# ColinWine/Multi-modal-Multi-label-Facial-Action-Unit-Detection-with-Transformer

Hardware: NVIDIA B200
Metric: AVFormer hot-path clips/sec (forward) (higher is better)
Workload: dtype bf16

## Files before the change

multi-modal-multi-label-facial-action-unit-detection-with-transformer_b200/csrc/avf_api.cu:

```cuda
#include <atomic>
#include <cstdarg>
#include <cstdio>
#include <cstring>

#include "avf_common.cuh"
#include "avf_internal.h"

namespace avf {

static thread_local char g_err[512] = "";
static std::atomic<uint64_t> g_launches{0};
static std::atomic<int> g_pdl{1};
bool pdl_enabled() { return g_pdl.load() != 0; }
static std::atomic<int> g_sm_cap{0};
int sm_cap() { return g_sm_cap.load(); }
static std::atomic<int> g_fused{1};

void count_launch() { g_launches.fetch_add(1, std::memory_order_relaxed); }

void set_error(const char* fmt, ...) {
  va_list ap;
  va_start(ap, fmt);
  vsnprintf(g_err, sizeof(g_err), fmt, ap);
  va_end(ap);
}

int check_cuda(cudaError_t e, const char* what) {
  if (e == cudaSuccess) return 0;
  set_error("CUDA error %d (%s) at %s", int(e), cudaGetErrorString(e), what);
  return int(e);
}

static int require_device() {
  static int state = 0;
  if (state == 0) {
    int n = 0;
    cudaError_t e = cudaGetDeviceCount(&n);
    if (e != cudaSuccess || n == 0) {
      cudaGetLastError();
      state = -1;
    } else {
      state = 1;
    }
  }
  if (state < 0) {
    set_error("no CUDA device: the AVFormer B200 path has no CPU fallback");
    return AVF_ENODEVICE;
  }
  return 0;
}

static bool tcgen05_ok() {
  static int state = 0;
  if (state == 0) {
    int dev = 0, major = 0;
    if (cudaGetDevice(&dev) == cudaSuccess && cudaDeviceGetAttribute(&major, cudaDevAttrComputeCapabilityMajor, dev) == cudaSuccess)
      state = (major == 10) ? 1 : -1;
    else
      state = -1;
  }
  return state > 0;
}

static inline size_t align_up(size_t v, size_t a = 256) { return (v + a - 1) / a * a; }
static inline size_t elt(int mode) { return mode == AVF_BF16 ? 2 : 4; }

struct EncoderWs {
  void* ln;
  void* qkv;
  void* attn;
  void* hid;
  size_t total;
};

static EncoderWs carve_encoder_ws(const avf_stack_shape* s, int mode, void* base) {
  const size_t R = size_t(s->n_seq) * s->n_tok, I = size_t(s->heads) * s->dim_head, e = elt(mode);
  uint8_t* p = static_cast<uint8_t*>(base);
  EncoderWs w;
  size_t off = 0;
  w.ln = p + off;   off += align_up(R * s->dim * e);
  w.qkv = p + off;  off += align_up(R * 3 * I * e);
  w.attn = p + off; off += align_up(R * I * e);
  w.hid = p + off;  off += align_up(R * s->mlp_dim * e);
  w.total = off;
  return w;
}

static int check_shape(const avf_stack_shape* s) {
  AVF_REQUIRE(s != nullptr, AVF_EINVAL, "null stack shape");
  AVF_REQUIRE(s->n_seq > 0 && s->n_tok > 0 && s->depth > 0, AVF_EINVAL, "empty stack: n_seq=%d n_tok=%d depth=%d", s->n_seq, s->n_tok, s->depth);
  AVF_REQUIRE(s->dim % 128 == 0 && s->dim <= 1536, AVF_EUNSUPPORTED, "dim=%d must be a multiple of 128 (<= 1536)", s->dim);
  AVF_REQUIRE(s->dim_head == 32 || s->dim_head == 64, AVF_EUNSUPPORTED, "dim_head=%d (supported: 32, 64)", s->dim_head);
  AVF_REQUIRE((s->heads * s->dim_head) % 64 == 0 && s->mlp_dim % 64 == 0, AVF_EUNSUPPORTED, "inner=%d / mlp=%d must be multiples of 64", s->heads * s->dim_head, s->mlp_dim);
  AVF_REQUIRE(s->n_tok <= 64 || s->dim_head == 64, AVF_EUNSUPPORTED,
              "n_tok=%d: sequences longer than 64 tokens are not part of this path for dim_head=%d", s->n_tok, s->dim_head);
  AVF_REQUIRE(s->n_tok <= 256, AVF_EUNSUPPORTED, "n_tok=%d: sequences longer than 256 tokens are not part of this path", s->n_tok);
  return 0;
}

int linear(int mode, const void* a, int lda, const void* w, const float* bias, const float* res, int ld_res, void* c, int ldc,
           int c_mode, int m, int n, int k, int flags, cudaStream_t st) {
  if (mode == AVF_BF16) {
    AVF_REQUIRE(tcgen05_ok(), AVF_EUNSUPPORTED, "bf16 mode needs an sm_100 device (tcgen05)");
    return linear_umma(a, lda, w, bias, res, ld_res, c, ldc, c_mode, m, n, k, flags, st);
  }
  return linear_f32(static_cast<const float*>(a), lda, static_cast<const float*>(w), bias, res, ld_res, c, ldc, c_mode, m, n, k, flags, st);
}

static bool fused_rows(int mode, const avf_stack_shape* s, int ld_x, const float* out, int ld_out) {
  return mode == AVF_BF16 && g_fused.load() && tcgen05_ok() && encoder_fused_supported(s) &&
         ld_x % 4 == 0 && (out == nullptr || ld_out % 4 == 0);
}

static int encoder_stack(int mode, const avf_stack_shape* s, const avf_layer_weights* L, float* x, int ld_x, float* out, int ld_out,
                         void* ws, size_t ws_bytes, cudaStream_t st, const uint8_t* keep = nullptr) {
  int e = check_shape(s);
  if (e) return e;
  AVF_REQUIRE(mode == AVF_BF16 || mode == AVF_FP32, AVF_EINVAL, "mode=%d", mode);
  AVF_REQUIRE(L != nullptr && x != nullptr && ws != nullptr, AVF_EINVAL, "null pointer argument");
  if (keep == nullptr && fused_rows(mode, s, ld_x, out, ld_out))
    return encoder_fused(1, s, L, x, ld_x, out ? out : x, out ? ld_out : ld_x, nullptr, nullptr, nullptr, nullptr, nullptr, st);
  const EncoderWs w = carve_encoder_ws(s, mode, ws);
  AVF_REQUIRE(ws_bytes >= w.total, AVF_EWORKSPACE, "workspace too small: %zu < %zu bytes", ws_bytes, w.total);
  const int R = s->n_seq * s->n_tok, D = s->dim, I = s->heads * s->dim_head, M = s->mlp_dim;
  for (int l = 0; l < s->depth; ++l) {
    const avf_layer_weights& W = L[l];
    if ((e = layernorm(mode, x, ld_x, W.ln1_gamma, W.ln1_beta, w.ln, R, D, st))) return e;
    if ((e = linear(mode, w.ln, D, W.w_qkv, nullptr, nullptr, 0, w.qkv, 3 * I, mode, R, 3 * I, D, 0, st))) return e;
    if ((e = attention_small(mode, w.qkv, w.attn, s->n_seq, s->n_tok, s->heads, s->dim_head, st, keep))) return e;
    if ((e = linear(mode, w.attn, I, W.w_out, W.b_out, x, ld_x, x, ld_x, AVF_FP32, R, D, I, AVF_EPI_BIAS | AVF_EPI_RESIDUAL, st))) return e;
    if ((e = layernorm(mode, x, ld_x, W.ln2_gamma, W.ln2_beta, w.ln, R, D, st))) return e;
    if ((e = linear(mode, w.ln, D, W.w_ff1, W.b_ff1, nullptr, 0, w.hid, M, mode, R, M, D, AVF_EPI_BIAS | AVF_EPI_GELU, st))) return e;
    const bool last = (l == s->depth - 1) && out != nullptr;
    if ((e = linear(mode, w.hid, M, W.w_ff2, W.b_ff2, x, ld_x, last ? out : x, last ? ld_out : ld_x, AVF_FP32, R, D, M,
                    AVF_EPI_BIAS | AVF_EPI_RESIDUAL, st)))
      return e;
  }
  return 0;
}

static int tformer_check(const avf_stack_shape* s, const avf_layer_weights* layers, const void* in, const float* cls_token, const float* pos,
                         const float* cls_out, const void* workspace, size_t workspace_bytes, size_t need) {
  int e = check_shape(s);
  if (e) return e;
  AVF_REQUIRE(layers && in && cls_token && pos && cls_out && workspace, AVF_EINVAL, "tformer_fwd: null pointer");
  AVF_REQUIRE(s->n_tok >= 2, AVF_EINVAL, "tformer_fwd: n_tok=%d (cls + at least one frame)", s->n_tok);
  AVF_REQUIRE(workspace_bytes >= need, AVF_EWORKSPACE, "workspace too small: %zu < %zu bytes", workspace_bytes, need);
  return 0;
}

static int tformer_layers(int mode, const avf_stack_shape* s, const avf_layer_weights* layers, void* workspace, float* cls_out, const uint8_t* keep,
                          cudaStream_t st) {
  int e = 0;
  const int B = s->n_seq, N = s->n_tok, R = B * N, D = s->dim, I = s->heads * s->dim_head, M = s->mlp_dim;
  uint8_t* p = static_cast<uint8_t*>(workspace);
  float* x = reinterpret_cast<float*>(p);   p += align_up(size_t(R) * D * 4);
  void* enc_ws = p;
  const EncoderWs w = carve_encoder_ws(s, mode, enc_ws);
  p += w.total;
  float* xc = reinterpret_cast<float*>(p);  p += align_up(size_t(B) * D * 4);
  void* lnc = p;                            p += align_up(size_t(B) * D * elt(mode));
  void* oc = p;                             p += align_up(size_t(B) * I * elt(mode));
  void* hc = p;
  if (s->depth > 1) {
    avf_stack_shape head = *s;
    head.depth = s->depth - 1;
    if ((e = encoder_stack(mode, &head, layers, x, D, nullptr, 0, enc_ws, w.total, st, keep))) return e;
  }
  const avf_layer_weights& W = layers[s->depth - 1];
  if ((e = layernorm(mode, x, D, W.ln1_gamma, W.ln1_beta, w.ln, R, D, st))) return e;
  if ((e = linear(mode, w.ln, D, W.w_qkv, nullptr, nullptr, 0, w.qkv, 3 * I, mode, R, 3 * I, D, 0, st))) return e;
  if (mode == AVF_BF16) {
    if ((e = attention_mma_bf16(w.qkv, oc, B, N, s->heads, s->dim_head, st, 1, keep))) return e;
  } else {
    if ((e = attention_small(mode, w.qkv, w.attn, B, N, s->heads, s->dim_head, st, keep))) return e;
    AVF_CUDA(cudaMemcpy2DAsync(oc, size_t(I) * 4, w.attn, size_t(N) * I * 4, size_t(I) * 4, B, cudaMemcpyDeviceToDevice, st));
  }
  if ((e = rows_gather(x, size_t(N) * D, xc, B, D, st))) return e;
  if ((e = linear(mode, oc, I, W.w_out, W.b_out, xc, D, xc, D, AVF_FP32, B, D, I, AVF_EPI_BIAS | AVF_EPI_RESIDUAL, st))) return e;
  if ((e = layernorm(mode, xc, D, W.ln2_gamma, W.ln2_beta, lnc, B, D, st))) return e;
  if ((e = linear(mode, lnc, D, W.w_ff1, W.b_ff1, nullptr, 0, hc, M, mode, B, M, D, AVF_EPI_BIAS | AVF_EPI_GELU, st))) return e;
  return linear(mode, hc, M, W.w_ff2, W.b_ff2, xc, D, cls_out, D, AVF_FP32, B, D, M, AVF_EPI_BIAS | AVF_EPI_RESIDUAL, st);
}

static int tformer_fwd(int mode, int io_mode, const avf_stack_shape* s, const avf_layer_weights* layers, const void* frames, const float* cls_token,
                       const float* pos, float* cls_out, void* workspace, size_t workspace_bytes, const uint8_t* keep, cudaStream_t st) {
  int e = tformer_check(s, layers, frames, cls_token, pos, cls_out, workspace, workspace_bytes, avf_tformer_workspace_bytes(s, mode));
  if (e) return e;
  if ((e = tformer_embed(io_mode, frames, cls_token, pos, static_cast<float*>(workspace), s->n_seq, s->n_tok - 1, s->dim, st))) return e;
  return tformer_layers(mode, s, layers, workspace, cls_out, keep, st);
}

static int tformer_fwd_indexed(int mode, int io_mode, const avf_stack_shape* s, const avf_layer_weights* layers, const void* bank, int n_bank,
                               const int32_t* index, const float* cls_token, const float* pos, float* cls_out, void* workspace, size_t workspace_bytes,
                               cudaStream_t st) {
  int e = tformer_check(s, layers, index, cls_token, pos, cls_out, workspace, workspace_bytes, avf_tformer_indexed_workspace_bytes(s, mode));
  if (e) return e;
  AVF_REQUIRE(n_bank >= 0 && (bank != nullptr || n_bank == 0), AVF_EINVAL, "tformer_fwd_indexed: bank of %d frames at %p", n_bank, bank);
  uint8_t* keep = static_cast<uint8_t*>(workspace) + avf_tformer_workspace_bytes(s, mode);
  if ((e = tformer_embed_indexed(io_mode, bank, n_bank, index, cls_token, pos, static_cast<float*>(workspace), keep, s->n_seq, s->n_tok - 1, s->dim, st)))
    return e;
  return tformer_layers(mode, s, layers, workspace, cls_out, keep, st);
}

}

using namespace avf;

extern "C" {

int avf_abi_version(void) { return AVF_ABI_VERSION; }

const char* avf_last_error(void) { return g_err; }

uint64_t avf_launch_count(void) { return g_launches.load(std::memory_order_relaxed); }

int avf_set_fused_enabled(int enabled) {
  const int old = g_fused.exchange(enabled ? 1 : 0);
  return old;
}

int avf_set_pdl_enabled(int enabled) { return g_pdl.exchange(enabled ? 1 : 0); }

int avf_set_sm_cap(int cap) { return g_sm_cap.exchange(cap > 0 ? cap : 0); }

int avf_encoder_fused_supported(const avf_stack_shape* s, int mode) {
  return (s != nullptr && mode == AVF_BF16 && s->n_seq > 0 && encoder_fused_supported(s)) ? 1 : 0;
}

int avf_debug_fused_prof(uint64_t* out64, int reset) { return fused_prof_read(reinterpret_cast<unsigned long long*>(out64), reset); }

int avf_debug_tmap_cache(uint64_t* hits, uint64_t* misses) {
  if (hits == nullptr || misses == nullptr) return AVF_EINVAL;
  tmap_cache_stats(hits, misses);
  return 0;
}

int avf_debug_gemm_prof(uint64_t* out16) { return gemm_prof_read(reinterpret_cast<unsigned long long*>(out16)); }

int avf_debug_set_trap_buffer(void* host_mapped_words) { return fused_set_trap_buffer(host_mapped_words); }

int avf_device_info(int32_t* sm_count, int32_t* cc, int32_t* has_tcgen05) {
  int e = require_device();
  if (e) return e;
  int dev = 0, sms = 0, major = 0, minor = 0;
  AVF_CUDA(cudaGetDevice(&dev));
  AVF_CUDA(cudaDeviceGetAttribute(&sms, cudaDevAttrMultiProcessorCount, dev));
  AVF_CUDA(cudaDeviceGetAttribute(&major, cudaDevAttrComputeCapabilityMajor, dev));
  AVF_CUDA(cudaDeviceGetAttribute(&minor, cudaDevAttrComputeCapabilityMinor, dev));
  if (sm_count) *sm_count = sms;
  if (cc) *cc = major * 10 + minor;
  if (has_tcgen05) *has_tcgen05 = major == 10 ? 1 : 0;
  return 0;
}

size_t avf_encoder_workspace_bytes(const avf_stack_shape* s, int mode) {
  if (s == nullptr || s->n_seq <= 0 || s->n_tok <= 0) return 0;
  return carve_encoder_ws(s, mode, nullptr).total;
}

int avf_encoder_stack_fwd(int mode, const avf_stack_shape* s, const avf_layer_weights* layers, float* x, int32_t ld_x, float* out,
                          int32_t ld_out, void* workspace, size_t workspace_bytes, void* stream) {
  int e = require_device();
  if (e) return e;
  return encoder_stack(mode, s, layers, x, ld_x, out, ld_out, workspace, workspace_bytes, static_cast<cudaStream_t>(stream));
}

int avf_encoder_stack_fwd_masked(int mode, const avf_stack_shape* s, const avf_layer_weights* layers, const uint8_t* keep, float* x, int32_t ld_x,
                                 float* out, int32_t ld_out, void* workspace, size_t workspace_bytes, void* stream) {
  int e = require_device();
  if (e) return e;
  return encoder_stack(mode, s, layers, x, ld_x, out, ld_out, workspace, workspace_bytes, static_cast<cudaStream_t>(stream), keep);
}

int avf_token_stack_fwd(int mode, const avf_stack_shape* s, const avf_layer_weights* layers, float* x, int32_t ld_x, const float* pos, float* out,
                        int32_t ld_out, const float* w_last, float* out21, int32_t* decisions, void* workspace, size_t workspace_bytes, void* stream) {
  int e = require_device();
  if (e) return e;
  if ((e = check_shape(s))) return e;
  AVF_REQUIRE(layers && x && workspace, AVF_EINVAL, "token_stack: null pointer");
  AVF_REQUIRE(w_last == nullptr || (s->n_tok == 12 && out21 != nullptr), AVF_EINVAL, "token_stack: AU logits need 12 tokens per clip and out21 (n_tok=%d)",
              s->n_tok);
  cudaStream_t st = static_cast<cudaStream_t>(stream);
  if (fused_rows(mode, s, ld_x, out, ld_out))
    return encoder_fused(1, s, layers, x, ld_x, (out || w_last) ? out : x, out ? ld_out : ld_x, pos, nullptr, w_last, out21, decisions, st);
  if (pos != nullptr && (e = add_row_periodic(x, ld_x, pos, s->n_seq * s->n_tok, s->dim, s->n_tok, st))) return e;
  if ((e = encoder_stack(mode, s, layers, x, ld_x, out, ld_out, workspace, workspace_bytes, st))) return e;
  return w_last == nullptr ? 0 : au_logits(out ? out : x, out ? ld_out : ld_x, w_last, out21, decisions, s->n_seq, s->dim, st);
}

int avf_layernorm_fwd(int out_mode, const float* x, int32_t ld_x, const float* gamma, const float* beta, void* y, int32_t rows,
                      int32_t dim, void* stream) {
  int e = require_device();
  if (e) return e;
  AVF_REQUIRE(x && gamma && beta && y, AVF_EINVAL, "layernorm: null pointer");
  return layernorm(out_mode, x, ld_x, gamma, beta, y, rows, dim, static_cast<cudaStream_t>(stream));
}

int avf_linear_fwd(int mode, const void* a, int32_t lda, const void* w, const float* bias, const float* residual, int32_t ld_res,
                   void* c, int32_t ldc, int c_mode, int32_t m, int32_t n, int32_t k, int epilogue_flags, void* stream) {
  int e = require_device();
  if (e) return e;
  AVF_REQUIRE(a && w && c, AVF_EINVAL, "linear: null pointer");
  AVF_REQUIRE(!(epilogue_flags & AVF_EPI_BIAS) || bias, AVF_EINVAL, "linear: bias flag without bias");
  AVF_REQUIRE(!(epilogue_flags & AVF_EPI_RESIDUAL) || residual, AVF_EINVAL, "linear: residual flag without residual");
  return linear(mode, a, lda, w, bias, residual, ld_res, c, ldc, c_mode, m, n, k, epilogue_flags, static_cast<cudaStream_t>(stream));
}

int avf_attention_fwd(int io_mode, const void* qkv, void* out, int32_t n_seq, int32_t n_tok, int32_t heads, int32_t dim_head, void* stream) {
  int e = require_device();
  if (e) return e;
  AVF_REQUIRE(qkv && out, AVF_EINVAL, "attention: null pointer");
  return attention_small(io_mode, qkv, out, n_seq, n_tok, heads, dim_head, static_cast<cudaStream_t>(stream));
}

int avf_attention_fwd_masked(int io_mode, const void* qkv, void* out, int32_t n_seq, int32_t n_tok, int32_t heads, int32_t dim_head, const uint8_t* keep,
                             void* stream) {
  int e = require_device();
  if (e) return e;
  AVF_REQUIRE(qkv && out, AVF_EINVAL, "attention: null pointer");
  return attention_small(io_mode, qkv, out, n_seq, n_tok, heads, dim_head, static_cast<cudaStream_t>(stream), keep);
}

int avf_sformer_tokens_pack(int io_mode, const void* fmap, const float* pos, float* x, int32_t n_frames, int32_t dim, int32_t hw, void* stream) {
  int e = require_device();
  if (e) return e;
  AVF_REQUIRE(fmap && x, AVF_EINVAL, "sformer_tokens_pack: null pointer");
  return sformer_pack(io_mode, fmap, pos, x, n_frames, dim, hw, static_cast<cudaStream_t>(stream));
}

int avf_sformer_tokens_unpack(int io_mode, const float* x, void* fmap, int32_t n_frames, int32_t dim, int32_t hw, void* stream) {
  int e = require_device();
  if (e) return e;
  AVF_REQUIRE(fmap && x, AVF_EINVAL, "sformer_tokens_unpack: null pointer");
  return sformer_unpack(io_mode, x, fmap, n_frames, dim, hw, static_cast<cudaStream_t>(stream));
}

size_t avf_sformer_workspace_bytes(const avf_stack_shape* s, int mode) {
  if (s == nullptr || s->n_seq <= 0 || s->n_tok <= 0) return 0;
  return align_up(size_t(s->n_seq) * s->n_tok * s->dim * 4) + carve_encoder_ws(s, mode, nullptr).total + align_up(encoder_fused_scratch_bytes());
}

int avf_sformer_fwd(int mode, int io_mode, const avf_stack_shape* s, const avf_layer_weights* layers, const float* pos,
                    const void* fmap_in, void* fmap_out, void* workspace, size_t workspace_bytes, void* stream) {
  int e = require_device();
  if (e) return e;
  if ((e = check_shape(s))) return e;
  AVF_REQUIRE(layers && pos && fmap_in && fmap_out && workspace, AVF_EINVAL, "sformer_fwd: null pointer");
  const size_t need = avf_sformer_workspace_bytes(s, mode);
  AVF_REQUIRE(workspace_bytes >= need, AVF_EWORKSPACE, "workspace too small: %zu < %zu bytes", workspace_bytes, need);
  cudaStream_t st = static_cast<cudaStream_t>(stream);
  if (mode == AVF_BF16 && io_mode == AVF_BF16 && g_fused.load() && tcgen05_ok() && encoder_fused_supported(s) && s->dim == 256)
    return encoder_fused(0, s, layers, fmap_in, 0, fmap_out, 0, pos, workspace, nullptr, nullptr, nullptr, st);
  float* x = static_cast<float*>(workspace);
  const size_t xbytes = align_up(size_t(s->n_seq) * s->n_tok * s->dim * 4);
  if ((e = sformer_pack(io_mode, fmap_in, pos, x, s->n_seq, s->dim, s->n_tok, st))) return e;
  if ((e = encoder_stack(mode, s, layers, x, s->dim, nullptr, 0, static_cast<uint8_t*>(workspace) + xbytes, workspace_bytes - xbytes, st))) return e;
  return sformer_unpack(io_mode, x, fmap_out, s->n_seq, s->dim, s->n_tok, st);
}

int avf_tformer_embed(int io_mode, const void* frames, const float* cls_token, const float* pos, float* x, int32_t n_clips,
                      int32_t n_frames, int32_t dim, void* stream) {
  int e = require_device();
  if (e) return e;
  AVF_REQUIRE(frames && cls_token && pos && x, AVF_EINVAL, "tformer_embed: null pointer");
  return tformer_embed(io_mode, frames, cls_token, pos, x, n_clips, n_frames, dim, static_cast<cudaStream_t>(stream));
}

size_t avf_tformer_workspace_bytes(const avf_stack_shape* s, int mode) {
  if (s == nullptr || s->n_seq <= 0 || s->n_tok <= 0) return 0;
  const size_t B = s->n_seq, D = s->dim, I = size_t(s->heads) * s->dim_head, M = s->mlp_dim, e = elt(mode);
  return align_up(B * s->n_tok * D * 4) + carve_encoder_ws(s, mode, nullptr).total + align_up(B * D * 4) + align_up(B * D * e) + align_up(B * I * e) +
         align_up(B * M * e);
}

int avf_tformer_fwd(int mode, int io_mode, const avf_stack_shape* s, const avf_layer_weights* layers, const void* frames,
                    const float* cls_token, const float* pos, float* cls_out, void* workspace, size_t workspace_bytes, void* stream) {
  int e = require_device();
  if (e) return e;
  return tformer_fwd(mode, io_mode, s, layers, frames, cls_token, pos, cls_out, workspace, workspace_bytes, nullptr, static_cast<cudaStream_t>(stream));
}

int avf_tformer_fwd_masked(int mode, int io_mode, const avf_stack_shape* s, const avf_layer_weights* layers, const uint8_t* keep, const void* frames,
                           const float* cls_token, const float* pos, float* cls_out, void* workspace, size_t workspace_bytes, void* stream) {
  int e = require_device();
  if (e) return e;
  return tformer_fwd(mode, io_mode, s, layers, frames, cls_token, pos, cls_out, workspace, workspace_bytes, keep, static_cast<cudaStream_t>(stream));
}

size_t avf_tformer_indexed_workspace_bytes(const avf_stack_shape* s, int mode) {
  if (s == nullptr || s->n_seq <= 0 || s->n_tok <= 0) return 0;
  return avf_tformer_workspace_bytes(s, mode) + align_up(size_t(s->n_seq) * s->n_tok);
}

int avf_tformer_fwd_indexed(int mode, int io_mode, const avf_stack_shape* s, const avf_layer_weights* layers, const void* bank, int32_t n_bank,
                            const int32_t* index, const float* cls_token, const float* pos, float* cls_out, void* workspace, size_t workspace_bytes,
                            void* stream) {
  int e = require_device();
  if (e) return e;
  return tformer_fwd_indexed(mode, io_mode, s, layers, bank, n_bank, index, cls_token, pos, cls_out, workspace, workspace_bytes,
                             static_cast<cudaStream_t>(stream));
}

int avf_tformer_embed_indexed(int io_mode, const void* bank, int32_t n_bank, const int32_t* index, const float* cls_token, const float* pos, float* x,
                              uint8_t* keep, int32_t n_clips, int32_t n_frames, int32_t dim, void* stream) {
  int e = require_device();
  if (e) return e;
  AVF_REQUIRE(index && cls_token && pos && x && keep, AVF_EINVAL, "tformer_embed_indexed: null pointer");
  AVF_REQUIRE(bank != nullptr || n_bank == 0, AVF_EINVAL, "tformer_embed_indexed: bank of %d frames at %p", n_bank, bank);
  return tformer_embed_indexed(io_mode, bank, n_bank, index, cls_token, pos, x, keep, n_clips, n_frames, dim, static_cast<cudaStream_t>(stream));
}

int avf_tformer_cls_extract(const float* x, float* cls, int32_t n_clips, int32_t n_tok, int32_t dim, void* stream) {
  int e = require_device();
  if (e) return e;
  AVF_REQUIRE(x && cls, AVF_EINVAL, "tformer_cls_extract: null pointer");
  return rows_gather(x, size_t(n_tok) * dim, cls, n_clips, dim, static_cast<cudaStream_t>(stream));
}

int avf_token_front_fwd(int mode, const float* emb, int32_t ld_emb, const float* bn_gamma, const float* bn_beta, const float* bn_mean,
                        const float* bn_var, const void* w_cat, const float* b_cat, const float* pos, float* x, int32_t n_clips,
                        int32_t in_dim, int32_t emb_dim, int32_t n_tok, void* workspace, size_t workspace_bytes, void* stream) {
  int e = require_device();
  if (e) return e;
  AVF_REQUIRE(emb && bn_gamma && bn_beta && bn_mean && bn_var && w_cat && b_cat && x && workspace, AVF_EINVAL, "token_front: null pointer");
  AVF_REQUIRE(n_clips > 0 && in_dim > 0 && emb_dim > 0 && n_tok > 0, AVF_EINVAL, "token_front: n_clips=%d n_tok=%d", n_clips, n_tok);
  const size_t need = align_up(size_t(n_clips) * in_dim * elt(mode));
  AVF_REQUIRE(workspace_bytes >= need, AVF_EWORKSPACE, "workspace too small: %zu < %zu bytes", workspace_bytes, need);
  cudaStream_t st = static_cast<cudaStream_t>(stream);
  if ((e = bn_rows(mode, emb, ld_emb, bn_gamma, bn_beta, bn_mean, bn_var, workspace, n_clips, in_dim, st))) return e;
  if ((e = linear(mode, workspace, in_dim, w_cat, b_cat, nullptr, 0, x, n_tok * emb_dim, AVF_FP32, n_clips, n_tok * emb_dim, in_dim, AVF_EPI_BIAS, st))) return e;
  return pos == nullptr ? 0 : add_row_periodic(x, emb_dim, pos, n_clips * n_tok, emb_dim, n_tok, st);
}

int avf_au_former_front_fwd(int mode, const float* emb, int32_t ld_emb, const float* bn_gamma, const float* bn_beta, const float* bn_mean,
                            const float* bn_var, const void* w_cat, const float* b_cat, const float* pos, float* x, int32_t n_clips,
                            int32_t in_dim, int32_t emb_dim, void* workspace, size_t workspace_bytes, void* stream) {
  return avf_token_front_fwd(mode, emb, ld_emb, bn_gamma, bn_beta, bn_mean, bn_var, w_cat, b_cat, pos, x, n_clips, in_dim, emb_dim, 12, workspace,
                             workspace_bytes, stream);
}

int avf_au_logits_fwd(const float* x, int32_t ld_x, const float* w_last, float* out21, int32_t* decisions, int32_t n_clips, int32_t dim, void* stream) {
  int e = require_device();
  if (e) return e;
  AVF_REQUIRE(x && w_last, AVF_EINVAL, "au_logits: null pointer");
  return au_logits(x, ld_x, w_last, out21, decisions, n_clips, dim, static_cast<cudaStream_t>(stream));
}

int avf_au_bce_loss(const float* logits, int32_t ld_logits, const float* labels, const float* pos_weight, float* loss_out, float* dlogits,
                    int32_t n_clips, void* stream) {
  int e = require_device();
  if (e) return e;
  AVF_REQUIRE(logits && labels && pos_weight && loss_out, AVF_EINVAL, "au_bce_loss: null pointer");
  return au_bce(logits, ld_logits, labels, pos_weight, loss_out, dlogits, n_clips, static_cast<cudaStream_t>(stream));
}

size_t avf_peer_gather_bytes(int32_t world, size_t n_floats) { return (world > 0 && world <= 1024) ? peer_gather_bytes(world, n_floats) : 0; }

int avf_logits_push(const float* logits, size_t n_floats, const uint64_t* peer_base, int32_t world, int32_t rank, const uint32_t* state, void* stream) {
  int e = require_device();
  if (e) return e;
  AVF_REQUIRE(logits && peer_base && state, AVF_EINVAL, "logits_push: null pointer");
  AVF_REQUIRE(world > 0 && world <= 1024 && rank >= 0 && rank < world && n_floats > 0, AVF_EINVAL, "logits_push: world %d rank %d n %zu", world, rank, n_floats);
  return logits_push(logits, n_floats, reinterpret_cast<const unsigned long long*>(peer_base), world, rank, state, static_cast<cudaStream_t>(stream));
}

int avf_logits_wait(const void* my_base, size_t n_floats, int32_t world, uint32_t* state, uint64_t timeout_ns, void* stream) {
  int e = require_device();
  if (e) return e;
  AVF_REQUIRE(my_base && state, AVF_EINVAL, "logits_wait: null pointer");
  AVF_REQUIRE(world > 0 && world <= 1024 && n_floats > 0, AVF_EINVAL, "logits_wait: world %d n %zu", world, n_floats);
  return logits_wait(my_base, n_floats, world, state, timeout_ns, static_cast<cudaStream_t>(stream));
}

size_t avf_peer_allreduce_bytes(int32_t world, size_t n_floats) { return (world > 0 && world <= 16) ? peer_allreduce_bytes(world, n_floats) : 0; }

int avf_grad_allreduce(const uint64_t* peer_base, size_t n_floats, int32_t world, int32_t rank, uint32_t* state, uint64_t timeout_ns, void* stream) {
  int e = require_device();
  if (e) return e;
  AVF_REQUIRE(peer_base && state, AVF_EINVAL, "grad_allreduce: null pointer");
  AVF_REQUIRE(world > 0 && world <= 16 && rank >= 0 && rank < world && n_floats > 0, AVF_EINVAL, "grad_allreduce: world %d (1..16) rank %d n %zu", world, rank, n_floats);
  return grad_allreduce(reinterpret_cast<const unsigned long long*>(peer_base), n_floats, world, rank, state, timeout_ns, static_cast<cudaStream_t>(stream));
}

int avf_adam_allreduce_step(const uint64_t* peer_base, size_t n_floats, int32_t world, int32_t rank, uint32_t* state, uint64_t timeout_ns, float* params,
                            float* exp_avg, float* exp_avg_sq, void* bf16_shadow, float lr, float beta1, float beta2, float eps, float weight_decay, int32_t step,
                            int decoupled, float grad_scale, void* stream) {
  int e = require_device();
  if (e) return e;
  AVF_REQUIRE(peer_base && state, AVF_EINVAL, "adam_allreduce_step: null pointer");
  AVF_REQUIRE(world > 0 && world <= 16 && rank >= 0 && rank < world && n_floats > 0, AVF_EINVAL, "adam_allreduce_step: world %d (1..16) rank %d n %zu", world, rank, n_floats);
  return adam_allreduce_step(reinterpret_cast<const unsigned long long*>(peer_base), n_floats, world, rank, state, timeout_ns, params, exp_avg, exp_avg_sq, bf16_shadow,
                             lr, beta1, beta2, eps, weight_decay, step, decoupled, grad_scale, static_cast<cudaStream_t>(stream));
}

int avf_au_confusion_update(const float* pred, int32_t ld_pred, float threshold, const float* labels, int32_t ld_labels, float ignore,
                            uint64_t* counts48, int32_t n_rows, void* stream) {
  int e = require_device();
  if (e) return e;
  return au_confusion(pred, ld_pred, threshold, labels, ld_labels, ignore, reinterpret_cast<unsigned long long*>(counts48), n_rows,
                      static_cast<cudaStream_t>(stream));
}

int avf_cast_f32_to_bf16(const float* src, void* dst, size_t n, void* stream) {
  int e = require_device();
  if (e) return e;
  AVF_REQUIRE((src && dst) || n == 0, AVF_EINVAL, "cast: null pointer");
  return cast_f32_bf16(src, dst, n, static_cast<cudaStream_t>(stream));
}

int avf_cast_bf16_to_f32(const void* src, float* dst, size_t n, void* stream) {
  int e = require_device();
  if (e) return e;
  AVF_REQUIRE((src && dst) || n == 0, AVF_EINVAL, "cast: null pointer");
  return cast_bf16_f32(src, dst, n, static_cast<cudaStream_t>(stream));
}

int avf_add_row_periodic(float* x, int32_t ld_x, const float* pos, int32_t rows, int32_t dim, int32_t period, void* stream) {
  int e = require_device();
  if (e) return e;
  AVF_REQUIRE(x && pos, AVF_EINVAL, "add_row_periodic: null pointer");
  return add_row_periodic(x, ld_x, pos, rows, dim, period, static_cast<cudaStream_t>(stream));
}

}
```

multi-modal-multi-label-facial-action-unit-detection-with-transformer_b200/csrc/avf_attention_mma.cu:

```cuda
#include "avf_common.cuh"
#include "avf_internal.h"

namespace avf {

namespace {

__device__ __forceinline__ void mma_bf16_16816(float (&d)[4], const uint32_t (&a)[4], uint32_t b0, uint32_t b1) {
  asm volatile(
      "mma.sync.aligned.m16n8k16.row.col.f32.bf16.bf16.f32 {%0,%1,%2,%3}, {%4,%5,%6,%7}, {%8,%9}, {%0,%1,%2,%3};"
      : "+f"(d[0]), "+f"(d[1]), "+f"(d[2]), "+f"(d[3])
      : "r"(a[0]), "r"(a[1]), "r"(a[2]), "r"(a[3]), "r"(b0), "r"(b1));
}

__device__ __forceinline__ void ldmatrix_x2_trans(uint32_t& r0, uint32_t& r1, const void* smem_row_ptr) {
  asm volatile("ldmatrix.sync.aligned.m8n8.x2.trans.shared.b16 {%0,%1}, [%2];" : "=r"(r0), "=r"(r1) : "r"(smem_u32(smem_row_ptr)));
}

__device__ __forceinline__ void quad_transpose32(uint32_t (&p)[4], int lane) {
  const bool b0 = lane & 1, b1 = lane & 2;
  uint32_t r;
  r = __shfl_xor_sync(0xffffffffu, b0 ? p[0] : p[1], 1); if (b0) p[0] = r; else p[1] = r;
  r = __shfl_xor_sync(0xffffffffu, b0 ? p[2] : p[3], 1); if (b0) p[2] = r; else p[3] = r;
  r = __shfl_xor_sync(0xffffffffu, b1 ? p[0] : p[2], 2); if (b1) p[0] = r; else p[2] = r;
  r = __shfl_xor_sync(0xffffffffu, b1 ? p[1] : p[3], 2); if (b1) p[1] = r; else p[3] = r;
}

__device__ __forceinline__ uint64_t keep_bits(const uint8_t* __restrict__ row, int n_tok, int lane) {
  const uint32_t lo = __ballot_sync(0xffffffffu, lane < n_tok && row[lane] != 0);
  const uint32_t hi = __ballot_sync(0xffffffffu, lane + 32 < n_tok && row[lane + 32] != 0);
  return (uint64_t(hi) << 32) | lo;
}

__device__ __forceinline__ float mask_score(float s, bool row_kept, uint64_t km, int c, int n_tok) {
  if (c >= n_tok) return -INFINITY;
  if (!row_kept) return 0.f;
  return ((km >> c) & 1) ? s : -INFINITY;
}

template <int DH, int NP, bool MASKED>
__global__ void __launch_bounds__(DH == 32 ? 128 : 64) attention_mma_kernel(const __nv_bfloat16* __restrict__ qkv, __nv_bfloat16* __restrict__ out,
                                                            int n_problems, int n_tok, int heads, float scale_log2e, int q_rows,
                                                            const uint8_t* __restrict__ keep) {
  pdl_wait();
  pdl_trigger();
  constexpr int PITCH = DH + 8;
  constexpr int WARPS = DH == 32 ? 4 : 2;
  __shared__ __align__(16) __nv_bfloat16 smem[WARPS][2][NP][PITCH];
  const int warp = threadIdx.x >> 5, lane = threadIdx.x & 31;
  const int prob = blockIdx.x * WARPS + warp;
  if (prob >= n_problems) return;
  const int seq = prob / heads, head = prob - seq * heads;
  const int inner = heads * DH;
  const size_t row0 = size_t(seq) * n_tok;
  const __nv_bfloat16* base = qkv + row0 * (3 * inner) + head * DH;
  __nv_bfloat16 (*Ks)[PITCH] = smem[warp][0];
  __nv_bfloat16 (*Vs)[PITCH] = smem[warp][1];
  uint64_t km = 0;
  if constexpr (MASKED) km = keep_bits(keep + row0, n_tok, lane);

  constexpr int CH = DH / 8;
  constexpr int NLD = NP * CH / 32;
  static_assert(NP * CH % 32 == 0, "whole warps of 16-byte chunks");
  uint4 kreg[NLD], vreg[NLD];
#pragma unroll
  for (int u = 0; u < NLD; ++u) {
    const int i = lane + u * 32, r = i / CH, c = i - r * CH;
    kreg[u] = make_uint4(0, 0, 0, 0);
    vreg[u] = make_uint4(0, 0, 0, 0);
    if (r < n_tok) {
      const __nv_bfloat16* p = base + size_t(r) * (3 * inner) + c * 8;
      kreg[u] = *reinterpret_cast<const uint4*>(p + inner);
      vreg[u] = *reinterpret_cast<const uint4*>(p + 2 * inner);
    }
  }
#pragma unroll
  for (int u = 0; u < NLD; ++u) {
    const int i = lane + u * 32, r = i / CH, c = i - r * CH;
    *reinterpret_cast<uint4*>(&Ks[r][c * 8]) = kreg[u];
    *reinterpret_cast<uint4*>(&Vs[r][c * 8]) = vreg[u];
  }
  __syncwarp();

  const int g = lane >> 2, t = lane & 3;
#pragma unroll 1
  for (int mt = 0; mt < NP / 16; ++mt) {
    if (mt * 16 >= q_rows) break;
    const int r_lo = mt * 16 + g, r_hi = r_lo + 8;
    uint32_t qf[DH / 16][4];
#pragma unroll
    for (int grp = 0; grp < DH / 32; ++grp) {
      uint32_t lo[4] = {0u, 0u, 0u, 0u}, hi[4] = {0u, 0u, 0u, 0u};
      if (r_lo < n_tok) {
        const uint4 v = *reinterpret_cast<const uint4*>(base + size_t(r_lo) * (3 * inner) + (grp * 4 + t) * 8);
        lo[0] = v.x; lo[1] = v.y; lo[2] = v.z; lo[3] = v.w;
      }
      if (r_hi < n_tok) {
        const uint4 v = *reinterpret_cast<const uint4*>(base + size_t(r_hi) * (3 * inner) + (grp * 4 + t) * 8);
        hi[0] = v.x; hi[1] = v.y; hi[2] = v.z; hi[3] = v.w;
      }
      quad_transpose32(lo, lane);
      quad_transpose32(hi, lane);
#pragma unroll
      for (int j = 0; j < 4; ++j) {
        const int ks = (grp * 4 + j) >> 1, half = (grp * 4 + j) & 1;
        qf[ks][half * 2] = lo[j];
        qf[ks][half * 2 + 1] = hi[j];
      }
    }
    float s[NP / 8][4];
#pragma unroll
    for (int nt = 0; nt < NP / 8; ++nt) {
      s[nt][0] = s[nt][1] = s[nt][2] = s[nt][3] = 0.f;
#pragma unroll
      for (int ks = 0; ks < DH / 16; ++ks) {
        const uint32_t b0 = *reinterpret_cast<const uint32_t*>(&Ks[nt * 8 + g][ks * 16 + 2 * t]);
        const uint32_t b1 = *reinterpret_cast<const uint32_t*>(&Ks[nt * 8 + g][ks * 16 + 8 + 2 * t]);
        mma_bf16_16816(s[nt], qf[ks], b0, b1);
      }
    }
    float m_lo = -INFINITY, m_hi = -INFINITY;
    const bool k_lo = (km >> r_lo) & 1, k_hi = (km >> r_hi) & 1;
#pragma unroll
    for (int nt = 0; nt < NP / 8; ++nt) {
      const int c = nt * 8 + 2 * t;
      if constexpr (MASKED) {
        s[nt][0] = mask_score(s[nt][0], k_lo, km, c, n_tok); s[nt][1] = mask_score(s[nt][1], k_lo, km, c + 1, n_tok);
        s[nt][2] = mask_score(s[nt][2], k_hi, km, c, n_tok); s[nt][3] = mask_score(s[nt][3], k_hi, km, c + 1, n_tok);
      } else {
        if (c >= n_tok) { s[nt][0] = -INFINITY; s[nt][2] = -INFINITY; }
        if (c + 1 >= n_tok) { s[nt][1] = -INFINITY; s[nt][3] = -INFINITY; }
      }
      m_lo = fmaxf(m_lo, fmaxf(s[nt][0], s[nt][1]));
      m_hi = fmaxf(m_hi, fmaxf(s[nt][2], s[nt][3]));
    }
    m_lo = fmaxf(m_lo, __shfl_xor_sync(0xffffffffu, m_lo, 1));
    m_lo = fmaxf(m_lo, __shfl_xor_sync(0xffffffffu, m_lo, 2));
    m_hi = fmaxf(m_hi, __shfl_xor_sync(0xffffffffu, m_hi, 1));
    m_hi = fmaxf(m_hi, __shfl_xor_sync(0xffffffffu, m_hi, 2));
    const float o_lo = m_lo * scale_log2e, o_hi = m_hi * scale_log2e;
    float l_lo = 0.f, l_hi = 0.f;
#pragma unroll
    for (int nt = 0; nt < NP / 8; ++nt) {
      s[nt][0] = exp2f(fmaf(s[nt][0], scale_log2e, -o_lo));
      s[nt][1] = exp2f(fmaf(s[nt][1], scale_log2e, -o_lo));
      s[nt][2] = exp2f(fmaf(s[nt][2], scale_log2e, -o_hi));
      s[nt][3] = exp2f(fmaf(s[nt][3], scale_log2e, -o_hi));
      l_lo += s[nt][0] + s[nt][1];
      l_hi += s[nt][2] + s[nt][3];
    }
    l_lo += __shfl_xor_sync(0xffffffffu, l_lo, 1);
    l_lo += __shfl_xor_sync(0xffffffffu, l_lo, 2);
    l_hi += __shfl_xor_sync(0xffffffffu, l_hi, 1);
    l_hi += __shfl_xor_sync(0xffffffffu, l_hi, 2);
    float o[DH / 8][4];
#pragma unroll
    for (int nt = 0; nt < DH / 8; ++nt) o[nt][0] = o[nt][1] = o[nt][2] = o[nt][3] = 0.f;
#pragma unroll
    for (int kt = 0; kt < NP / 16; ++kt) {
      uint32_t pa[4];
      pa[0] = pack_bf16x2(s[2 * kt][0], s[2 * kt][1]);
      pa[1] = pack_bf16x2(s[2 * kt][2], s[2 * kt][3]);
      pa[2] = pack_bf16x2(s[2 * kt + 1][0], s[2 * kt + 1][1]);
      pa[3] = pack_bf16x2(s[2 * kt + 1][2], s[2 * kt + 1][3]);
#pragma unroll
      for (int nt = 0; nt < DH / 8; ++nt) {
        uint32_t b0, b1;
        ldmatrix_x2_trans(b0, b1, &Vs[kt * 16 + (lane & 15)][nt * 8]);
        mma_bf16_16816(o[nt], pa, b0, b1);
      }
    }
    const float i_lo = 1.f / l_lo, i_hi = 1.f / l_hi;
    __nv_bfloat16* olo = out + (size_t(seq) * q_rows + r_lo) * inner + head * DH;
    __nv_bfloat16* ohi = out + (size_t(seq) * q_rows + r_hi) * inner + head * DH;
#pragma unroll
    for (int grp = 0; grp < DH / 32; ++grp) {
      uint32_t lo[4], hi[4];
#pragma unroll
      for (int j = 0; j < 4; ++j) {
        lo[j] = pack_bf16x2(o[grp * 4 + j][0] * i_lo, o[grp * 4 + j][1] * i_lo);
        hi[j] = pack_bf16x2(o[grp * 4 + j][2] * i_hi, o[grp * 4 + j][3] * i_hi);
      }
      quad_transpose32(lo, lane);
      quad_transpose32(hi, lane);
      if (r_lo < q_rows) *reinterpret_cast<uint4*>(olo + (grp * 4 + t) * 8) = make_uint4(lo[0], lo[1], lo[2], lo[3]);
      if (r_hi < q_rows) *reinterpret_cast<uint4*>(ohi + (grp * 4 + t) * 8) = make_uint4(hi[0], hi[1], hi[2], hi[3]);
    }
  }
}

template <int DH, int NP, bool MASKED>
int launch(const void* qkv, void* out, int n_seq, int n_tok, int heads, int q_rows, const uint8_t* keep, cudaStream_t st) {
  const int n_problems = n_seq * heads;
  const float scale_log2e = 1.4426950408889634f / sqrtf(float(DH));
  constexpr int kWarps = DH == 32 ? 4 : 2;
  launch_pdl(attention_mma_kernel<DH, NP, MASKED>, ceil_div(n_problems, kWarps), kWarps * 32, 0, st, static_cast<const __nv_bfloat16*>(qkv), static_cast<__nv_bfloat16*>(out),
                                                                      n_problems, n_tok, heads, scale_log2e, q_rows, keep);
  AVF_LAUNCH_CHECK("attention_mma_kernel");
  return 0;
}

template <int DH, int NP>
struct BwdCfg {
  static constexpr int PITCH = DH + 8;
  static constexpr int SLAB_BYTES = 4 * NP * PITCH * 2 + 3 * NP * 4;
  static constexpr int WARPS = SLAB_BYTES * 2 <= 46 * 1024 ? 2 : 1;
};

template <int DH, int NP, bool MASKED>
__global__ void __launch_bounds__(BwdCfg<DH, NP>::WARPS * 32) attention_bwd_mma_kernel(const __nv_bfloat16* __restrict__ qkv,
                                                                                       const __nv_bfloat16* __restrict__ dout,
                                                                                       __nv_bfloat16* __restrict__ dqkv, int n_problems,
                                                                                       int n_tok, int heads, float scale,
                                                                                       const uint8_t* __restrict__ keep) {
  pdl_wait();
  pdl_trigger();
  using Cfg = BwdCfg<DH, NP>;
  constexpr int PITCH = Cfg::PITCH, WARPS = Cfg::WARPS;
  __shared__ __align__(16) __nv_bfloat16 smem[WARPS][4][NP][PITCH];
  __shared__ float stats[WARPS][3][NP];
  const int warp = threadIdx.x >> 5, lane = threadIdx.x & 31;
  const int prob = blockIdx.x * WARPS + warp;
  if (prob >= n_problems) return;
  const int seq = prob / heads, head = prob - seq * heads;
  const int inner = heads * DH;
  const size_t row0 = size_t(seq) * n_tok;
  const __nv_bfloat16* base = qkv + row0 * (3 * inner) + head * DH;
  const __nv_bfloat16* dobase = dout + row0 * inner + head * DH;
  __nv_bfloat16* dbase = dqkv + row0 * (3 * inner) + head * DH;
  __nv_bfloat16 (*Qs)[PITCH] = smem[warp][0];
  __nv_bfloat16 (*Ks)[PITCH] = smem[warp][1];
  __nv_bfloat16 (*Vs)[PITCH] = smem[warp][2];
  __nv_bfloat16 (*Os)[PITCH] = smem[warp][3];
  float* st_m = stats[warp][0];
  float* st_il = stats[warp][1];
  float* st_d = stats[warp][2];
  const float scale_log2e = scale * 1.4426950408889634f;
  uint64_t km = 0;
  if constexpr (MASKED) km = keep_bits(keep + row0, n_tok, lane);

  constexpr int CH = DH / 8;
  for (int i = lane; i < NP * CH; i += 32) {
    const int r = i / CH, c = i - r * CH;
    uint4 q = make_uint4(0, 0, 0, 0), k = q, v = q, o = q;
    if (r < n_tok) {
      const __nv_bfloat16* p = base + size_t(r) * (3 * inner) + c * 8;
      q = *reinterpret_cast<const uint4*>(p);
      k = *reinterpret_cast<const uint4*>(p + inner);
      v = *reinterpret_cast<const uint4*>(p + 2 * inner);
      o = *reinterpret_cast<const uint4*>(dobase + size_t(r) * inner + c * 8);
    }
    *reinterpret_cast<uint4*>(&Qs[r][c * 8]) = q;
    *reinterpret_cast<uint4*>(&Ks[r][c * 8]) = k;
    *reinterpret_cast<uint4*>(&Vs[r][c * 8]) = v;
    *reinterpret_cast<uint4*>(&Os[r][c * 8]) = o;
  }
  __syncwarp();

  const int g = lane >> 2, t = lane & 3;
  auto load_a = [&](uint32_t (&f)[DH / 16][4], __nv_bfloat16 (*M)[PITCH], int r_lo) {
#pragma unroll
    for (int ks = 0; ks < DH / 16; ++ks) {
      f[ks][0] = *reinterpret_cast<const uint32_t*>(&M[r_lo][ks * 16 + 2 * t]);
      f[ks][1] = *reinterpret_cast<const uint32_t*>(&M[r_lo + 8][ks * 16 + 2 * t]);
      f[ks][2] = *reinterpret_cast<const uint32_t*>(&M[r_lo][ks * 16 + 8 + 2 * t]);
      f[ks][3] = *reinterpret_cast<const uint32_t*>(&M[r_lo + 8][ks * 16 + 8 + 2 * t]);
    }
  };
  auto mma_abt = [&](float (&c)[NP / 8][4], const uint32_t (&a)[DH / 16][4], __nv_bfloat16 (*M)[PITCH]) {
#pragma unroll
    for (int nt = 0; nt < NP / 8; ++nt) {
      c[nt][0] = c[nt][1] = c[nt][2] = c[nt][3] = 0.f;
#pragma unroll
      for (int ks = 0; ks < DH / 16; ++ks) {
        const uint32_t b0 = *reinterpret_cast<const uint32_t*>(&M[nt * 8 + g][ks * 16 + 2 * t]);
        const uint32_t b1 = *reinterpret_cast<const uint32_t*>(&M[nt * 8 + g][ks * 16 + 8 + 2 * t]);
        mma_bf16_16816(c[nt], a[ks], b0, b1);
      }
    }
  };
  auto mma_xm = [&](float (&d)[DH / 8][4], const float (&x)[NP / 8][4], __nv_bfloat16 (*M)[PITCH]) {
#pragma unroll
    for (int nt = 0; nt < DH / 8; ++nt) d[nt][0] = d[nt][1] = d[nt][2] = d[nt][3] = 0.f;
#pragma unroll
    for (int kt = 0; kt < NP / 16; ++kt) {
      uint32_t pa[4];
      pa[0] = pack_bf16x2(x[2 * kt][0], x[2 * kt][1]);
      pa[1] = pack_bf16x2(x[2 * kt][2], x[2 * kt][3]);
      pa[2] = pack_bf16x2(x[2 * kt + 1][0], x[2 * kt + 1][1]);
      pa[3] = pack_bf16x2(x[2 * kt + 1][2], x[2 * kt + 1][3]);
#pragma unroll
      for (int nt = 0; nt < DH / 8; ++nt) {
        uint32_t b0, b1;
        ldmatrix_x2_trans(b0, b1, &M[kt * 16 + (lane & 15)][nt * 8]);
        mma_bf16_16816(d[nt], pa, b0, b1);
      }
    }
  };
  auto store_rows = [&](const float (&d)[DH / 8][4], __nv_bfloat16* dst_col0, int r_lo, float mul) {
    __nv_bfloat16* lo = dst_col0 + size_t(r_lo) * (3 * inner) + 2 * t;
    __nv_bfloat16* hi = lo + size_t(8) * (3 * inner);
#pragma unroll
    for (int nt = 0; nt < DH / 8; ++nt) {
      if (r_lo < n_tok) *reinterpret_cast<uint32_t*>(lo + nt * 8) = pack_bf16x2(d[nt][0] * mul, d[nt][1] * mul);
      if (r_lo + 8 < n_tok) *reinterpret_cast<uint32_t*>(hi + nt * 8) = pack_bf16x2(d[nt][2] * mul, d[nt][3] * mul);
    }
  };

#pragma unroll 1
  for (int mt = 0; mt < NP / 16; ++mt) {
    if (mt * 16 >= n_tok) break;
    const int r_lo = mt * 16 + g;
    uint32_t af[DH / 16][4];
    float s[NP / 8][4], dp[NP / 8][4];
    load_a(af, Qs, r_lo);
    mma_abt(s, af, Ks);
    load_a(af, Os, r_lo);
    mma_abt(dp, af, Vs);
    float m_lo = -INFINITY, m_hi = -INFINITY;
    const bool k_lo = (km >> r_lo) & 1, k_hi = (km >> (r_lo + 8)) & 1;
#pragma unroll
    for (int nt = 0; nt < NP / 8; ++nt) {
      const int c = nt * 8 + 2 * t;
      if constexpr (MASKED) {
        s[nt][0] = mask_score(s[nt][0], k_lo, km, c, n_tok); s[nt][1] = mask_score(s[nt][1], k_lo, km, c + 1, n_tok);
        s[nt][2] = mask_score(s[nt][2], k_hi, km, c, n_tok); s[nt][3] = mask_score(s[nt][3], k_hi, km, c + 1, n_tok);
      } else {
        if (c >= n_tok) { s[nt][0] = -INFINITY; s[nt][2] = -INFINITY; }
        if (c + 1 >= n_tok) { s[nt][1] = -INFINITY; s[nt][3] = -INFINITY; }
      }
      m_lo = fmaxf(m_lo, fmaxf(s[nt][0], s[nt][1]));
      m_hi = fmaxf(m_hi, fmaxf(s[nt][2], s[nt][3]));
    }
    m_lo = fmaxf(m_lo, __shfl_xor_sync(0xffffffffu, m_lo, 1));
    m_lo = fmaxf(m_lo, __shfl_xor_sync(0xffffffffu, m_lo, 2));
    m_hi = fmaxf(m_hi, __shfl_xor_sync(0xffffffffu, m_hi, 1));
    m_hi = fmaxf(m_hi, __shfl_xor_sync(0xffffffffu, m_hi, 2));
    const float o_lo = m_lo * scale_log2e, o_hi = m_hi * scale_log2e;
    float l_lo = 0.f, l_hi = 0.f;
#pragma unroll
    for (int nt = 0; nt < NP / 8; ++nt) {
      s[nt][0] = exp2f(fmaf(s[nt][0], scale_log2e, -o_lo));
      s[nt][1] = exp2f(fmaf(s[nt][1], scale_log2e, -o_lo));
      s[nt][2] = exp2f(fmaf(s[nt][2], scale_log2e, -o_hi));
      s[nt][3] = exp2f(fmaf(s[nt][3], scale_log2e, -o_hi));
      l_lo += s[nt][0] + s[nt][1];
      l_hi += s[nt][2] + s[nt][3];
    }
    l_lo += __shfl_xor_sync(0xffffffffu, l_lo, 1);
    l_lo += __shfl_xor_sync(0xffffffffu, l_lo, 2);
    l_hi += __shfl_xor_sync(0xffffffffu, l_hi, 1);
    l_hi += __shfl_xor_sync(0xffffffffu, l_hi, 2);
    const float i_lo = 1.f / l_lo, i_hi = 1.f / l_hi;
    float d_lo = 0.f, d_hi = 0.f;
#pragma unroll
    for (int nt = 0; nt < NP / 8; ++nt) {
      s[nt][0] *= i_lo; s[nt][1] *= i_lo; s[nt][2] *= i_hi; s[nt][3] *= i_hi;
      d_lo += s[nt][0] * dp[nt][0] + s[nt][1] * dp[nt][1];
      d_hi += s[nt][2] * dp[nt][2] + s[nt][3] * dp[nt][3];
    }
    d_lo += __shfl_xor_sync(0xffffffffu, d_lo, 1);
    d_lo += __shfl_xor_sync(0xffffffffu, d_lo, 2);
    d_hi += __shfl_xor_sync(0xffffffffu, d_hi, 1);
    d_hi += __shfl_xor_sync(0xffffffffu, d_hi, 2);
    if (t == 0) {
      st_m[r_lo] = o_lo; st_il[r_lo] = i_lo; st_d[r_lo] = d_lo;
      st_m[r_lo + 8] = o_hi; st_il[r_lo + 8] = i_hi; st_d[r_lo + 8] = d_hi;
    }
#pragma unroll
    for (int nt = 0; nt < NP / 8; ++nt) {
      s[nt][0] *= dp[nt][0] - d_lo; s[nt][1] *= dp[nt][1] - d_lo;
      s[nt][2] *= dp[nt][2] - d_hi; s[nt][3] *= dp[nt][3] - d_hi;
      if constexpr (MASKED) {
        if (!k_lo) s[nt][0] = s[nt][1] = 0.f;
        if (!k_hi) s[nt][2] = s[nt][3] = 0.f;
      }
    }
    float dq[DH / 8][4];
    mma_xm(dq, s, Ks);
    store_rows(dq, dbase, r_lo, scale);
  }
  __syncwarp();

#pragma unroll 1
  for (int mt = 0; mt < NP / 16; ++mt) {
    if (mt * 16 >= n_tok) break;
    const int r_lo = mt * 16 + g;
    uint32_t af[DH / 16][4];
    float p[NP / 8][4], dp[NP / 8][4];
    load_a(af, Ks, r_lo);
    mma_abt(p, af, Qs);
    load_a(af, Vs, r_lo);
    mma_abt(dp, af, Os);
    float ds[NP / 8][4];
    const bool k_lo = (km >> r_lo) & 1, k_hi = (km >> (r_lo + 8)) & 1;
#pragma unroll
    for (int nt = 0; nt < NP / 8; ++nt) {
#pragma unroll
      for (int e = 0; e < 2; ++e) {
        const int qi = nt * 8 + 2 * t + e;
        const bool ok = qi < n_tok;
        const float m = ok ? st_m[qi] : 0.f, il = ok ? st_il[qi] : 0.f, dl = ok ? st_d[qi] : 0.f;
        float p0, p1;
        if constexpr (MASKED) {
          const bool qk = (km >> qi) & 1;
          p0 = ok ? exp2f(fmaf(qk ? (k_lo ? p[nt][e] : -INFINITY) : 0.f, scale_log2e, -m)) * il : 0.f;
          p1 = ok ? exp2f(fmaf(qk ? (k_hi ? p[nt][e + 2] : -INFINITY) : 0.f, scale_log2e, -m)) * il : 0.f;
          ds[nt][e] = qk ? p0 * (dp[nt][e] - dl) : 0.f;
          ds[nt][e + 2] = qk ? p1 * (dp[nt][e + 2] - dl) : 0.f;
        } else {
          p0 = ok ? exp2f(fmaf(p[nt][e], scale_log2e, -m)) * il : 0.f;
          p1 = ok ? exp2f(fmaf(p[nt][e + 2], scale_log2e, -m)) * il : 0.f;
          ds[nt][e] = p0 * (dp[nt][e] - dl);
          ds[nt][e + 2] = p1 * (dp[nt][e + 2] - dl);
        }
        p[nt][e] = p0;
        p[nt][e + 2] = p1;
      }
    }
    float acc[DH / 8][4];
    mma_xm(acc, p, Os);
    store_rows(acc, dbase + 2 * inner, r_lo, 1.f);
    mma_xm(acc, ds, Qs);
    store_rows(acc, dbase + inner, r_lo, scale);
  }
}

template <int DH, int NP, bool MASKED>
int launch_bwd(const void* qkv, const void* dout, void* dqkv, int n_seq, int n_tok, int heads, const uint8_t* keep, cudaStream_t st) {
  const int n_problems = n_seq * heads;
  constexpr int kWarps = BwdCfg<DH, NP>::WARPS;
  launch_pdl(attention_bwd_mma_kernel<DH, NP, MASKED>, ceil_div(n_problems, kWarps), kWarps * 32, 0, st, static_cast<const __nv_bfloat16*>(qkv), static_cast<const __nv_bfloat16*>(dout), static_cast<__nv_bfloat16*>(dqkv), n_problems, n_tok, heads,
      1.0f / sqrtf(float(DH)), keep);
  AVF_LAUNCH_CHECK("attention_bwd_mma_kernel");
  return 0;
}

constexpr int kLongDH = 64, kLongPitch = kLongDH + 8, kLongWarps = 8, kLongMaxTok = 256;
using LongRow = __nv_bfloat16[kLongPitch];

__host__ __device__ __forceinline__ int long_rows(int n_tok) { return (n_tok + 63) & ~63; }

__device__ __forceinline__ void keep_words(const uint8_t* __restrict__ row, int n_tok, uint64_t* km, int warp, int lane) {
  if (warp < 4) {
    const int b = warp * 64;
    const uint64_t w = keep_bits(row + b, min(max(n_tok - b, 0), 64), lane);
    if (lane == 0) km[warp] = w;
  }
}
__device__ __forceinline__ bool keep_bit(const uint64_t* km, int i) { return (km[i >> 6] >> (i & 63)) & 1; }

__device__ __forceinline__ void stage_rows(LongRow* dst, const __nv_bfloat16* __restrict__ src, size_t ld, int n_tok) {
  const int n = long_rows(n_tok) * (kLongDH / 8);
  for (int i = threadIdx.x; i < n; i += blockDim.x) {
    const int r = i >> 3, c = (i & 7) * 8;
    uint4 v = make_uint4(0, 0, 0, 0);
    if (r < n_tok) v = *reinterpret_cast<const uint4*>(src + size_t(r) * ld + c);
    *reinterpret_cast<uint4*>(&dst[r][c]) = v;
  }
}

__device__ __forceinline__ void long_load_a(uint32_t (&f)[4][4], const LongRow* M, int r_lo, int t) {
#pragma unroll
  for (int ks = 0; ks < 4; ++ks) {
    f[ks][0] = *reinterpret_cast<const uint32_t*>(&M[r_lo][ks * 16 + 2 * t]);
    f[ks][1] = *reinterpret_cast<const uint32_t*>(&M[r_lo + 8][ks * 16 + 2 * t]);
    f[ks][2] = *reinterpret_cast<const uint32_t*>(&M[r_lo][ks * 16 + 8 + 2 * t]);
    f[ks][3] = *reinterpret_cast<const uint32_t*>(&M[r_lo + 8][ks * 16 + 8 + 2 * t]);
  }
}
__device__ __forceinline__ void long_mma_abt(float (&c)[8][4], const uint32_t (&a)[4][4], const LongRow* M, int g, int t) {
#pragma unroll
  for (int nt = 0; nt < 8; ++nt) {
    c[nt][0] = c[nt][1] = c[nt][2] = c[nt][3] = 0.f;
#pragma unroll
    for (int ks = 0; ks < 4; ++ks) {
      const uint32_t b0 = *reinterpret_cast<const uint32_t*>(&M[nt * 8 + g][ks * 16 + 2 * t]);
      const uint32_t b1 = *reinterpret_cast<const uint32_t*>(&M[nt * 8 + g][ks * 16 + 8 + 2 * t]);
      mma_bf16_16816(c[nt], a[ks], b0, b1);
    }
  }
}
__device__ __forceinline__ void long_mma_xm(float (&d)[8][4], const float (&x)[8][4], const LongRow* M, int lane) {
#pragma unroll
  for (int kt = 0; kt < 4; ++kt) {
    uint32_t pa[4];
    pa[0] = pack_bf16x2(x[2 * kt][0], x[2 * kt][1]);
    pa[1] = pack_bf16x2(x[2 * kt][2], x[2 * kt][3]);
    pa[2] = pack_bf16x2(x[2 * kt + 1][0], x[2 * kt + 1][1]);
    pa[3] = pack_bf16x2(x[2 * kt + 1][2], x[2 * kt + 1][3]);
#pragma unroll
    for (int nt = 0; nt < 8; ++nt) {
      uint32_t b0, b1;
      ldmatrix_x2_trans(b0, b1, &M[kt * 16 + (lane & 15)][nt * 8]);
      mma_bf16_16816(d[nt], pa, b0, b1);
    }
  }
}
template <bool MASKED>
__device__ __forceinline__ void long_mask(float (&s)[8][4], bool k_lo, bool k_hi, uint64_t kw, int n_left, int t) {
#pragma unroll
  for (int nt = 0; nt < 8; ++nt) {
    const int c = nt * 8 + 2 * t;
    if constexpr (MASKED) {
      s[nt][0] = mask_score(s[nt][0], k_lo, kw, c, n_left); s[nt][1] = mask_score(s[nt][1], k_lo, kw, c + 1, n_left);
      s[nt][2] = mask_score(s[nt][2], k_hi, kw, c, n_left); s[nt][3] = mask_score(s[nt][3], k_hi, kw, c + 1, n_left);
    } else {
      if (c >= n_left) { s[nt][0] = -INFINITY; s[nt][2] = -INFINITY; }
      if (c + 1 >= n_left) { s[nt][1] = -INFINITY; s[nt][3] = -INFINITY; }
    }
  }
}
__device__ __forceinline__ float quad_max(float v) {
  v = fmaxf(v, __shfl_xor_sync(0xffffffffu, v, 1));
  return fmaxf(v, __shfl_xor_sync(0xffffffffu, v, 2));
}
__device__ __forceinline__ float quad_sum(float v) {
  v += __shfl_xor_sync(0xffffffffu, v, 1);
  return v + __shfl_xor_sync(0xffffffffu, v, 2);
}
__device__ __forceinline__ void long_store(const float (&d)[8][4], __nv_bfloat16* dst, size_t ld, int r_lo, int n_valid, float mul_lo, float mul_hi,
                                           int t) {
  __nv_bfloat16* lo = dst + size_t(r_lo) * ld + 2 * t;
  __nv_bfloat16* hi = lo + 8 * ld;
#pragma unroll
  for (int nt = 0; nt < 8; ++nt) {
    if (r_lo < n_valid) *reinterpret_cast<uint32_t*>(lo + nt * 8) = pack_bf16x2(d[nt][0] * mul_lo, d[nt][1] * mul_lo);
    if (r_lo + 8 < n_valid) *reinterpret_cast<uint32_t*>(hi + nt * 8) = pack_bf16x2(d[nt][2] * mul_hi, d[nt][3] * mul_hi);
  }
}

template <bool MASKED>
__global__ void __launch_bounds__(kLongWarps * 32) attention_long_mma_kernel(const __nv_bfloat16* __restrict__ qkv, __nv_bfloat16* __restrict__ out,
                                                                            int n_tok, int heads, float scale_log2e, int q_rows,
                                                                            const uint8_t* __restrict__ keep) {
  pdl_wait();
  pdl_trigger();
  extern __shared__ __align__(16) uint8_t smem_long[];
  const int NR = long_rows(n_tok);
  LongRow* Ks = reinterpret_cast<LongRow*>(smem_long);
  LongRow* Vs = Ks + NR;
  uint64_t* km = reinterpret_cast<uint64_t*>(Vs + NR);
  const int seq = blockIdx.x / heads, head = blockIdx.x - seq * heads;
  const int inner = heads * kLongDH, warp = threadIdx.x >> 5, lane = threadIdx.x & 31;
  const size_t row0 = size_t(seq) * n_tok, ld = size_t(3) * inner;
  const __nv_bfloat16* base = qkv + row0 * ld + head * kLongDH;
  stage_rows(Ks, base + inner, ld, n_tok);
  stage_rows(Vs, base + 2 * inner, ld, n_tok);
  if constexpr (MASKED) keep_words(keep + row0, n_tok, km, warp, lane);
  __syncthreads();

  const int g = lane >> 2, t = lane & 3, nkb = NR / 64;
#pragma unroll 1
  for (int mt = warp; mt * 16 < q_rows; mt += kLongWarps) {
    const int r_lo = mt * 16 + g, r_hi = r_lo + 8;
    uint32_t qf[4][4];
#pragma unroll
    for (int ks = 0; ks < 4; ++ks) {
#pragma unroll
      for (int h = 0; h < 2; ++h) {
        const int c = ks * 16 + h * 8 + 2 * t;
        qf[ks][2 * h] = r_lo < n_tok ? *reinterpret_cast<const uint32_t*>(base + size_t(r_lo) * ld + c) : 0u;
        qf[ks][2 * h + 1] = r_hi < n_tok ? *reinterpret_cast<const uint32_t*>(base + size_t(r_hi) * ld + c) : 0u;
      }
    }
    const bool k_lo = MASKED && keep_bit(km, r_lo), k_hi = MASKED && keep_bit(km, r_hi);
    float s[8][4];
    float m_lo = -INFINITY, m_hi = -INFINITY;
#pragma unroll 1
    for (int kb = 0; kb < nkb; ++kb) {
      long_mma_abt(s, qf, Ks + kb * 64, g, t);
      long_mask<MASKED>(s, k_lo, k_hi, MASKED ? km[kb] : 0, n_tok - kb * 64, t);
#pragma unroll
      for (int nt = 0; nt < 8; ++nt) {
        m_lo = fmaxf(m_lo, fmaxf(s[nt][0], s[nt][1]));
        m_hi = fmaxf(m_hi, fmaxf(s[nt][2], s[nt][3]));
      }
    }
    const float o_lo = quad_max(m_lo) * scale_log2e, o_hi = quad_max(m_hi) * scale_log2e;
    float l_lo = 0.f, l_hi = 0.f, o[8][4];
#pragma unroll
    for (int nt = 0; nt < 8; ++nt) o[nt][0] = o[nt][1] = o[nt][2] = o[nt][3] = 0.f;
#pragma unroll 1
    for (int kb = 0; kb < nkb; ++kb) {
      long_mma_abt(s, qf, Ks + kb * 64, g, t);
      long_mask<MASKED>(s, k_lo, k_hi, MASKED ? km[kb] : 0, n_tok - kb * 64, t);
#pragma unroll
      for (int nt = 0; nt < 8; ++nt) {
        s[nt][0] = exp2f(fmaf(s[nt][0], scale_log2e, -o_lo));
        s[nt][1] = exp2f(fmaf(s[nt][1], scale_log2e, -o_lo));
        s[nt][2] = exp2f(fmaf(s[nt][2], scale_log2e, -o_hi));
        s[nt][3] = exp2f(fmaf(s[nt][3], scale_log2e, -o_hi));
        l_lo += s[nt][0] + s[nt][1];
        l_hi += s[nt][2] + s[nt][3];
      }
      long_mma_xm(o, s, Vs + kb * 64, lane);
    }
    long_store(o, out + size_t(seq) * q_rows * inner + head * kLongDH, inner, r_lo, q_rows, 1.f / quad_sum(l_lo), 1.f / quad_sum(l_hi), t);
  }
}

template <bool MASKED>
__global__ void __launch_bounds__(kLongWarps * 32) attention_bwd_long_mma_kernel(const __nv_bfloat16* __restrict__ qkv,
                                                                                const __nv_bfloat16* __restrict__ dout,
                                                                                __nv_bfloat16* __restrict__ dqkv, int n_tok, int heads,
                                                                                float scale, const uint8_t* __restrict__ keep) {
  pdl_wait();
  pdl_trigger();
  extern __shared__ __align__(16) uint8_t smem_long[];
  const int NR = long_rows(n_tok);
  LongRow* Qs = reinterpret_cast<LongRow*>(smem_long);
  LongRow* Ks = Qs + NR;
  LongRow* Vs = Ks + NR;
  LongRow* Os = Vs + NR;
  float* st_m = reinterpret_cast<float*>(Os + NR);
  float* st_il = st_m + NR;
  float* st_d = st_il + NR;
  uint64_t* km = reinterpret_cast<uint64_t*>(st_d + NR);
  const int seq = blockIdx.x / heads, head = blockIdx.x - seq * heads;
  const int inner = heads * kLongDH, warp = threadIdx.x >> 5, lane = threadIdx.x & 31;
  const size_t row0 = size_t(seq) * n_tok, ld = size_t(3) * inner;
  const __nv_bfloat16* base = qkv + row0 * ld + head * kLongDH;
  __nv_bfloat16* dbase = dqkv + row0 * ld + head * kLongDH;
  stage_rows(Qs, base, ld, n_tok);
  stage_rows(Ks, base + inner, ld, n_tok);
  stage_rows(Vs, base + 2 * inner, ld, n_tok);
  stage_rows(Os, dout + row0 * inner + head * kLongDH, inner, n_tok);
  if constexpr (MASKED) keep_words(keep + row0, n_tok, km, warp, lane);
  __syncthreads();
  const float scale_log2e = scale * 1.4426950408889634f;
  const int g = lane >> 2, t = lane & 3, nkb = NR / 64;

#pragma unroll 1
  for (int mt = warp; mt * 16 < n_tok; mt += kLongWarps) {
    const int r_lo = mt * 16 + g, r_hi = r_lo + 8;
    uint32_t qf[4][4], of[4][4];
    long_load_a(qf, Qs, r_lo, t);
    long_load_a(of, Os, r_lo, t);
    const bool k_lo = MASKED && keep_bit(km, r_lo), k_hi = MASKED && keep_bit(km, r_hi);
    float s[8][4], dp[8][4];
    float m_lo = -INFINITY, m_hi = -INFINITY;
#pragma unroll 1
    for (int kb = 0; kb < nkb; ++kb) {
      long_mma_abt(s, qf, Ks + kb * 64, g, t);
      long_mask<MASKED>(s, k_lo, k_hi, MASKED ? km[kb] : 0, n_tok - kb * 64, t);
#pragma unroll
      for (int nt = 0; nt < 8; ++nt) {
        m_lo = fmaxf(m_lo, fmaxf(s[nt][0], s[nt][1]));
        m_hi = fmaxf(m_hi, fmaxf(s[nt][2], s[nt][3]));
      }
    }
    const float o_lo = quad_max(m_lo) * scale_log2e, o_hi = quad_max(m_hi) * scale_log2e;
    float l_lo = 0.f, l_hi = 0.f, e_lo = 0.f, e_hi = 0.f;
#pragma unroll 1
    for (int kb = 0; kb < nkb; ++kb) {
      long_mma_abt(s, qf, Ks + kb * 64, g, t);
      long_mask<MASKED>(s, k_lo, k_hi, MASKED ? km[kb] : 0, n_tok - kb * 64, t);
      long_mma_abt(dp, of, Vs + kb * 64, g, t);
#pragma unroll
      for (int nt = 0; nt < 8; ++nt) {
        const float a0 = exp2f(fmaf(s[nt][0], scale_log2e, -o_lo)), a1 = exp2f(fmaf(s[nt][1], scale_log2e, -o_lo));
        const float a2 = exp2f(fmaf(s[nt][2], scale_log2e, -o_hi)), a3 = exp2f(fmaf(s[nt][3], scale_log2e, -o_hi));
        l_lo += a0 + a1;
        l_hi += a2 + a3;
        e_lo += a0 * dp[nt][0] + a1 * dp[nt][1];
        e_hi += a2 * dp[nt][2] + a3 * dp[nt][3];
      }
    }
    const float i_lo = 1.f / quad_sum(l_lo), i_hi = 1.f / quad_sum(l_hi);
    const float d_lo = quad_sum(e_lo) * i_lo, d_hi = quad_sum(e_hi) * i_hi;
    if (t == 0) {
      st_m[r_lo] = o_lo; st_il[r_lo] = i_lo; st_d[r_lo] = d_lo;
      st_m[r_hi] = o_hi; st_il[r_hi] = i_hi; st_d[r_hi] = d_hi;
    }
    float dq[8][4];
#pragma unroll
    for (int nt = 0; nt < 8; ++nt) dq[nt][0] = dq[nt][1] = dq[nt][2] = dq[nt][3] = 0.f;
#pragma unroll 1
    for (int kb = 0; kb < nkb; ++kb) {
      long_mma_abt(s, qf, Ks + kb * 64, g, t);
      long_mask<MASKED>(s, k_lo, k_hi, MASKED ? km[kb] : 0, n_tok - kb * 64, t);
      long_mma_abt(dp, of, Vs + kb * 64, g, t);
#pragma unroll
      for (int nt = 0; nt < 8; ++nt) {
        s[nt][0] = exp2f(fmaf(s[nt][0], scale_log2e, -o_lo)) * i_lo * (dp[nt][0] - d_lo);
        s[nt][1] = exp2f(fmaf(s[nt][1], scale_log2e, -o_lo)) * i_lo * (dp[nt][1] - d_lo);
        s[nt][2] = exp2f(fmaf(s[nt][2], scale_log2e, -o_hi)) * i_hi * (dp[nt][2] - d_hi);
        s[nt][3] = exp2f(fmaf(s[nt][3], scale_log2e, -o_hi)) * i_hi * (dp[nt][3] - d_hi);
        if constexpr (MASKED) {
          if (!k_lo) s[nt][0] = s[nt][1] = 0.f;
          if (!k_hi) s[nt][2] = s[nt][3] = 0.f;
        }
      }
      long_mma_xm(dq, s, Ks + kb * 64, lane);
    }
    long_store(dq, dbase, ld, r_lo, n_tok, scale, scale, t);
  }
  __syncthreads();

#pragma unroll 1
  for (int mt = warp; mt * 16 < n_tok; mt += kLongWarps) {
    const int r_lo = mt * 16 + g;
    uint32_t kf[4][4], vf[4][4];
    long_load_a(kf, Ks, r_lo, t);
    long_load_a(vf, Vs, r_lo, t);
    const bool k_lo = MASKED && keep_bit(km, r_lo), k_hi = MASKED && keep_bit(km, r_lo + 8);
    float dv[8][4], dk[8][4];
#pragma unroll
    for (int nt = 0; nt < 8; ++nt) dv[nt][0] = dv[nt][1] = dv[nt][2] = dv[nt][3] = dk[nt][0] = dk[nt][1] = dk[nt][2] = dk[nt][3] = 0.f;
#pragma unroll 1
    for (int qb = 0; qb < nkb; ++qb) {
      float p[8][4], ds[8][4];
      long_mma_abt(p, kf, Qs + qb * 64, g, t);
      long_mma_abt(ds, vf, Os + qb * 64, g, t);
      const uint64_t qw = MASKED ? km[qb] : 0;
#pragma unroll
      for (int nt = 0; nt < 8; ++nt) {
#pragma unroll
        for (int e = 0; e < 2; ++e) {
          const int ql = nt * 8 + 2 * t + e, qi = qb * 64 + ql;
          const bool ok = qi < n_tok;
          const float m = ok ? st_m[qi] : 0.f, il = ok ? st_il[qi] : 0.f, dl = ok ? st_d[qi] : 0.f;
          float p0, p1;
          if constexpr (MASKED) {
            const bool qk = (qw >> ql) & 1;
            p0 = ok ? exp2f(fmaf(qk ? (k_lo ? p[nt][e] : -INFINITY) : 0.f, scale_log2e, -m)) * il : 0.f;
            p1 = ok ? exp2f(fmaf(qk ? (k_hi ? p[nt][e + 2] : -INFINITY) : 0.f, scale_log2e, -m)) * il : 0.f;
            ds[nt][e] = qk ? p0 * (ds[nt][e] - dl) : 0.f;
            ds[nt][e + 2] = qk ? p1 * (ds[nt][e + 2] - dl) : 0.f;
          } else {
            p0 = ok ? exp2f(fmaf(p[nt][e], scale_log2e, -m)) * il : 0.f;
            p1 = ok ? exp2f(fmaf(p[nt][e + 2], scale_log2e, -m)) * il : 0.f;
            ds[nt][e] = p0 * (ds[nt][e] - dl);
            ds[nt][e + 2] = p1 * (ds[nt][e + 2] - dl);
          }
          p[nt][e] = p0;
          p[nt][e + 2] = p1;
        }
      }
      long_mma_xm(dv, p, Os + qb * 64, lane);
      long_mma_xm(dk, ds, Qs + qb * 64, lane);
    }
    long_store(dv, dbase + 2 * inner, ld, r_lo, n_tok, 1.f, 1.f, t);
    long_store(dk, dbase + inner, ld, r_lo, n_tok, scale, scale, t);
  }
}

size_t long_fwd_smem(int n_tok) { return size_t(2) * long_rows(n_tok) * kLongPitch * 2 + 4 * sizeof(uint64_t); }
size_t long_bwd_smem(int n_tok) { return size_t(4) * long_rows(n_tok) * kLongPitch * 2 + size_t(3) * long_rows(n_tok) * 4 + 4 * sizeof(uint64_t); }

template <bool MASKED>
int launch_long(const void* qkv, void* out, int n_seq, int n_tok, int heads, int q_rows, const uint8_t* keep, cudaStream_t st) {
  auto kern = attention_long_mma_kernel<MASKED>;
  static PerDeviceOnce once;
  if (once.first()) {
    AVF_CUDA(cudaFuncSetAttribute(kern, cudaFuncAttributeMaxDynamicSharedMemorySize, int(long_fwd_smem(kLongMaxTok))));
  }
  launch_pdl(kern, n_seq * heads, kLongWarps * 32, long_fwd_smem(n_tok), st, static_cast<const __nv_bfloat16*>(qkv), static_cast<__nv_bfloat16*>(out), n_tok,
             heads, 1.4426950408889634f / sqrtf(float(kLongDH)), q_rows, keep);
  AVF_LAUNCH_CHECK("attention_long_mma_kernel");
  return 0;
}

template <bool MASKED>
int launch_bwd_long(const void* qkv, const void* dout, void* dqkv, int n_seq, int n_tok, int heads, const uint8_t* keep, cudaStream_t st) {
  auto kern = attention_bwd_long_mma_kernel<MASKED>;
  static PerDeviceOnce once;
  if (once.first()) {
    AVF_CUDA(cudaFuncSetAttribute(kern, cudaFuncAttributeMaxDynamicSharedMemorySize, int(long_bwd_smem(kLongMaxTok))));
  }
  launch_pdl(kern, n_seq * heads, kLongWarps * 32, long_bwd_smem(n_tok), st, static_cast<const __nv_bfloat16*>(qkv), static_cast<const __nv_bfloat16*>(dout),
             static_cast<__nv_bfloat16*>(dqkv), n_tok, heads, 1.0f / sqrtf(float(kLongDH)), keep);
  AVF_LAUNCH_CHECK("attention_bwd_long_mma_kernel");
  return 0;
}

}

int attention_mma_bf16(const void* qkv, void* out, int n_seq, int n_tok, int heads, int dim_head, cudaStream_t st, int q_rows, const uint8_t* keep) {
  AVF_REQUIRE(n_tok >= 1 && n_tok <= kLongMaxTok && (n_tok <= 64 || dim_head == kLongDH), AVF_EUNSUPPORTED,
              "attention: n_tok=%d with dim_head=%d (1..64 tokens; 64-wide heads up to 256)", n_tok, dim_head);
  if (q_rows <= 0 || q_rows > n_tok) q_rows = n_tok;
  if (n_tok > 64)
    return keep ? launch_long<true>(qkv, out, n_seq, n_tok, heads, q_rows, keep, st) : launch_long<false>(qkv, out, n_seq, n_tok, heads, q_rows, nullptr, st);
  const int np = (n_tok + 15) / 16 * 16;
#define AVF_ATT(D, P)                                                                                   \
  if (dim_head == D && np == P)                                                                         \
    return keep ? launch<D, P, true>(qkv, out, n_seq, n_tok, heads, q_rows, keep, st)                   \
                : launch<D, P, false>(qkv, out, n_seq, n_tok, heads, q_rows, nullptr, st);
  AVF_ATT(32, 16) AVF_ATT(32, 32) AVF_ATT(32, 48) AVF_ATT(32, 64)
  AVF_ATT(64, 16) AVF_ATT(64, 32) AVF_ATT(64, 48) AVF_ATT(64, 64)
#undef AVF_ATT
  AVF_REQUIRE(false, AVF_EUNSUPPORTED, "attention: dim_head=%d (supported: 32, 64)", dim_head);
  return 0;
}

}

namespace avf {
int attention_bwd_mma_bf16(const void* qkv, const void* dout, void* dqkv, int n_seq, int n_tok, int heads, int dim_head, cudaStream_t st,
                           const uint8_t* keep) {
  AVF_REQUIRE(n_tok >= 1 && n_tok <= kLongMaxTok && (n_tok <= 64 || dim_head == kLongDH), AVF_EUNSUPPORTED,
              "attention_bwd: n_tok=%d with dim_head=%d (1..64 tokens; 64-wide heads up to 256)", n_tok, dim_head);
  if (n_tok > 64)
    return keep ? launch_bwd_long<true>(qkv, dout, dqkv, n_seq, n_tok, heads, keep, st)
                : launch_bwd_long<false>(qkv, dout, dqkv, n_seq, n_tok, heads, nullptr, st);
  const int np = (n_tok + 15) / 16 * 16;
#define AVF_ATT(D, P)                                                                                   \
  if (dim_head == D && np == P)                                                                         \
    return keep ? launch_bwd<D, P, true>(qkv, dout, dqkv, n_seq, n_tok, heads, keep, st)                \
                : launch_bwd<D, P, false>(qkv, dout, dqkv, n_seq, n_tok, heads, nullptr, st);
  AVF_ATT(32, 16) AVF_ATT(32, 32) AVF_ATT(32, 48) AVF_ATT(32, 64)
  AVF_ATT(64, 16) AVF_ATT(64, 32) AVF_ATT(64, 48) AVF_ATT(64, 64)
#undef AVF_ATT
  AVF_REQUIRE(false, AVF_EUNSUPPORTED, "attention_bwd: dim_head=%d (supported: 32, 64)", dim_head);
  return 0;
}
}
```

multi-modal-multi-label-facial-action-unit-detection-with-transformer_b200/csrc/avf_gemm_umma.cu:

```cuda
#include <cuda.h>

#include <atomic>
#include <unordered_map>

#include <algorithm>
#include <mutex>

#include "avf_common.cuh"

namespace avf {

namespace {

constexpr int BM = 128;
constexpr int BK = 64;
constexpr int UMMA_K = 16;

template <int BN, int STAGES>
struct GemmCfg {
  static constexpr int A_BYTES = BM * BK * 2;
  static constexpr int W_BYTES = BN * BK * 2;
  static constexpr int STAGE_BYTES = A_BYTES + W_BYTES;
  static constexpr int BAR_OFF = STAGES * STAGE_BYTES;
  static constexpr int BIAS_OFF = BAR_OFF + 256;
  static constexpr int SMEM_BYTES = BIAS_OFF + 2 * BN * 4 + 1024;
  static constexpr int TMEM_COLS = 2 * BN;
};

__device__ __forceinline__ void quad_transpose(uint4 (&p)[4], int lane) {
  auto xchg = [&](uint4& keep_lo, uint4& keep_hi, bool upper, int mask) {
    uint4 snd = upper ? keep_lo : keep_hi, rcv;
    rcv.x = __shfl_xor_sync(0xffffffffu, snd.x, mask);
    rcv.y = __shfl_xor_sync(0xffffffffu, snd.y, mask);
    rcv.z = __shfl_xor_sync(0xffffffffu, snd.z, mask);
    rcv.w = __shfl_xor_sync(0xffffffffu, snd.w, mask);
    if (upper) keep_lo = rcv; else keep_hi = rcv;
  };
  const bool b0 = lane & 1, b1 = lane & 2;
  xchg(p[0], p[1], b0, 1);
  xchg(p[2], p[3], b0, 1);
  xchg(p[0], p[2], b1, 2);
  xchg(p[1], p[3], b1, 2);
}

__device__ __forceinline__ void quad_load16(const float* src, int ld, int row, int col, int M, int lane, float4 (&out)[4]) {
  const int row_q = row - (lane & 3);
  uint4 p[4];
#pragma unroll
  for (int i = 0; i < 4; ++i)
    p[i] = row_q + i < M ? *reinterpret_cast<const uint4*>(src + size_t(row_q + i) * ld + col + (lane & 3) * 4) : make_uint4(0u, 0u, 0u, 0u);
  quad_transpose(p, lane);
#pragma unroll
  for (int j = 0; j < 4; ++j) out[j] = make_float4(__uint_as_float(p[j].x), __uint_as_float(p[j].y), __uint_as_float(p[j].z), __uint_as_float(p[j].w));
}

template <typename OutT>
__device__ __forceinline__ void epilogue_chunk(const uint32_t (&v)[32], int row, int col0, OutT* C, int ldc,
                                               const float* __restrict__ bias, const float* res, int ld_res, int flags,
                                               __nv_bfloat16* aux, int ld_aux, const DropSpec& drop, int n_total, int M,
                                               const float4* pre_res = nullptr) {
  const bool valid = row < M;
  const int lane = threadIdx.x & 31;
  float f[32];
#pragma unroll
  for (int j = 0; j < 32; ++j) f[j] = __uint_as_float(v[j]);
  if ((flags & AVF_EPI_DGELU) && valid) {
    const __nv_bfloat16* ap = aux + size_t(row) * ld_aux + col0;
#pragma unroll
    for (int j = 0; j < 32; j += 8) {
      const uint4 pk = *reinterpret_cast<const uint4*>(ap + j);
      const uint32_t w[4] = {pk.x, pk.y, pk.z, pk.w};
#pragma unroll
      for (int q = 0; q < 4; ++q) {
        f[j + 2 * q] *= gelu_tanh_grad(__uint_as_float(w[q] << 16));
        f[j + 2 * q + 1] *= gelu_tanh_grad(__uint_as_float(w[q] & 0xffff0000u));
      }
    }
  }
  if (flags & AVF_EPI_BIAS) {
#pragma unroll
    for (int j = 0; j < 32; j += 4) {
      const float4 b = *reinterpret_cast<const float4*>(bias + col0 + j);
      f[j] += b.x; f[j + 1] += b.y; f[j + 2] += b.z; f[j + 3] += b.w;
    }
  }
  if ((flags & AVF_EPI_SAVE_PRE) && valid) {
    __nv_bfloat16* ap = aux + size_t(row) * ld_aux + col0;
#pragma unroll
    for (int j = 0; j < 32; j += 8) {
      uint4 o;
      o.x = pack_bf16x2(f[j], f[j + 1]);
      o.y = pack_bf16x2(f[j + 2], f[j + 3]);
      o.z = pack_bf16x2(f[j + 4], f[j + 5]);
      o.w = pack_bf16x2(f[j + 6], f[j + 7]);
      *reinterpret_cast<uint4*>(ap + j) = o;
    }
  }
  if (flags & AVF_EPI_GELU) {
#pragma unroll
    for (int j = 0; j < 32; ++j) f[j] = gelu_tanh<true>(f[j]);
  }
  if (flags & AVF_EPI_DROPOUT) {
    const uint32_t i0 = uint32_t(row) * uint32_t(n_total) + uint32_t(col0);
#pragma unroll
    for (int j = 0; j < 32; ++j) f[j] *= drop_factor(drop, i0 + j);
  }
  if (flags & AVF_EPI_RESIDUAL) {
    float4 r8[8];
    if (pre_res == nullptr) {
      quad_load16(res, ld_res, row, col0, M, lane, reinterpret_cast<float4(&)[4]>(r8[0]));
      quad_load16(res, ld_res, row, col0 + 16, M, lane, reinterpret_cast<float4(&)[4]>(r8[4]));
    }
#pragma unroll
    for (int j = 0; j < 32; j += 4) {
      const float4 r = pre_res != nullptr ? pre_res[j >> 2] : r8[j >> 2];
      f[j] += r.x; f[j + 1] += r.y; f[j + 2] += r.z; f[j + 3] += r.w;
    }
  }
  const int row_q = row - (lane & 3);
  if constexpr (sizeof(OutT) == 4) {
#pragma unroll
    for (int h = 0; h < 2; ++h) {
      uint4 p[4];
#pragma unroll
      for (int j = 0; j < 4; ++j)
        p[j] = make_uint4(__float_as_uint(f[h * 16 + 4 * j]), __float_as_uint(f[h * 16 + 4 * j + 1]), __float_as_uint(f[h * 16 + 4 * j + 2]),
                          __float_as_uint(f[h * 16 + 4 * j + 3]));
      quad_transpose(p, lane);
#pragma unroll
      for (int i = 0; i < 4; ++i)
        if (row_q + i < M) *reinterpret_cast<uint4*>(reinterpret_cast<float*>(C) + size_t(row_q + i) * ldc + col0 + h * 16 + (lane & 3) * 4) = p[i];
    }
  } else {
    uint4 p[4];
#pragma unroll
    for (int j = 0; j < 4; ++j) {
      p[j].x = pack_bf16x2(f[8 * j], f[8 * j + 1]);
      p[j].y = pack_bf16x2(f[8 * j + 2], f[8 * j + 3]);
      p[j].z = pack_bf16x2(f[8 * j + 4], f[8 * j + 5]);
      p[j].w = pack_bf16x2(f[8 * j + 6], f[8 * j + 7]);
    }
    quad_transpose(p, lane);
#pragma unroll
    for (int i = 0; i < 4; ++i)
      if (row_q + i < M) *reinterpret_cast<uint4*>(reinterpret_cast<__nv_bfloat16*>(C) + size_t(row_q + i) * ldc + col0 + (lane & 3) * 8) = p[i];
  }
}

#ifdef AVF_GEMM_PROF
__device__ unsigned long long g_gemm_prof[16];
__device__ __forceinline__ void gprof(int i) {
  if (blockIdx.x == 0) {
    unsigned long long t;
    asm volatile("mov.u64 %0, %%globaltimer;" : "=l"(t));
    g_gemm_prof[i] = t;
  }
}
#else
__device__ __forceinline__ void gprof(int) {}
#endif

template <int BN, int STAGES, typename OutT, bool A_MN, bool B_MN>
__global__ void __launch_bounds__(384, 1)
gemm_umma_kernel(const __grid_constant__ CUtensorMap tm_a, const __grid_constant__ CUtensorMap tm_w,
                 OutT* C, int ldc, const float* __restrict__ bias,
                 const float* res, int ld_res, int M, int N, int K, int flags,
                 __nv_bfloat16* aux, int ld_aux, int splits, size_t split_stride, DropSpec drop) {
  using Cfg = GemmCfg<BN, STAGES>;
  extern __shared__ uint8_t smem_raw[];
  uint8_t* smem = reinterpret_cast<uint8_t*>((reinterpret_cast<uintptr_t>(smem_raw) + 1023) & ~uintptr_t(1023));
  uint64_t* full_bar = reinterpret_cast<uint64_t*>(smem + Cfg::BAR_OFF);
  uint64_t* empty_bar = full_bar + STAGES;
  uint64_t* acc_full = empty_bar + STAGES;
  uint64_t* acc_empty = acc_full + 2;
  uint32_t* tmem_slot = reinterpret_cast<uint32_t*>(acc_empty + 2);

  const int warp = threadIdx.x >> 5, lane = threadIdx.x & 31;
  if (threadIdx.x == 0) gprof(0);
  const int kblocks_total = (K + BK - 1) / BK;
  const int kb_per_split = (kblocks_total + splits - 1) / splits;
  const int n_blocks = N / BN;
  const int mn_tiles = n_blocks * ((M + BM - 1) / BM);
  const int n_tiles = mn_tiles * splits;

  if (warp == 0 && lane == 0) {
    tma_prefetch_desc(&tm_a);
    tma_prefetch_desc(&tm_w);
    for (int s = 0; s < STAGES; ++s) {
      mbar_init(&full_bar[s], 1);
      mbar_init(&empty_bar[s], 1);
    }
    for (int b = 0; b < 2; ++b) {
      mbar_init(&acc_full[b], 1);
      mbar_init(&acc_empty[b], 8);
    }
    fence_barrier_init();
  }
  if (warp == 2) {
    tmem_alloc(tmem_slot, Cfg::TMEM_COLS);
    tmem_relinquish();
  }
  tc_fence_before();
  __syncthreads();
  tc_fence_after();
  const uint32_t tmem_base = *tmem_slot;
  if (threadIdx.x == 0) gprof(1);
  pdl_wait();
  pdl_trigger();
  if (threadIdx.x == 0) gprof(2);

  if (warp == 0) {
    const bool leader = elect_one();
    {
      uint32_t it = 0;
      for (int tile = blockIdx.x; tile < n_tiles; tile += gridDim.x) {
        const int split = tile / mn_tiles, mn = tile - split * mn_tiles;
        const int m0 = (mn / n_blocks) * BM, n0 = (mn % n_blocks) * BN;
        const int kb0 = split * kb_per_split, kb1 = min(kblocks_total, kb0 + kb_per_split);
        for (int kb = kb0; kb < kb1; ++kb, ++it) {
          const int s = it % STAGES;
          const uint32_t ph = (it / STAGES) & 1;
          mbar_wait(&empty_bar[s], ph ^ 1);
          uint8_t* st = smem + s * Cfg::STAGE_BYTES;
          if (leader) {
            mbar_expect_tx(&full_bar[s], Cfg::STAGE_BYTES);
            if constexpr (A_MN) {
#pragma unroll
              for (int p = 0; p < BM / 64; ++p) tma_load_2d(st + p * 8192, &tm_a, &full_bar[s], m0 + p * 64, kb * BK);
            } else {
              tma_load_2d(st, &tm_a, &full_bar[s], kb * BK, m0);
            }
            if constexpr (B_MN) {
#pragma unroll
              for (int p = 0; p < BN / 64; ++p) tma_load_2d(st + Cfg::A_BYTES + p * 8192, &tm_w, &full_bar[s], n0 + p * 64, kb * BK);
            } else {
              tma_load_2d(st + Cfg::A_BYTES, &tm_w, &full_bar[s], kb * BK, n0);
            }
          }
          __syncwarp();
        }
      }
    }
  } else if (warp == 1) {
    const bool leader = elect_one();
    {
      constexpr uint32_t idesc = make_idesc_bf16(BM, BN, A_MN ? 1 : 0, B_MN ? 1 : 0);
      uint32_t it = 0, lt = 0;
      for (int tile = blockIdx.x; tile < n_tiles; tile += gridDim.x, ++lt) {
        const uint32_t buf = lt & 1, aph = (lt >> 1) & 1;
        mbar_wait(&acc_empty[buf], aph ^ 1);
        tc_fence_after();
        const uint32_t tmem_d = tmem_base + buf * BN;
        const int split = tile / mn_tiles;
        const int kb0 = split * kb_per_split, kb1 = min(kblocks_total, kb0 + kb_per_split);
        for (int kb = kb0; kb < kb1; ++kb, ++it) {
          const int s = it % STAGES;
          const uint32_t ph = (it / STAGES) & 1;
          mbar_wait(&full_bar[s], ph);
          tc_fence_after();
          if (leader && it == 0) gprof(3);
          const uint32_t a_addr = smem_u32(smem + s * Cfg::STAGE_BYTES);
          const uint64_t da = A_MN ? make_desc(a_addr, 8192, 1024, 2) : make_desc_sw128_kmajor(a_addr);
          const uint64_t db = B_MN ? make_desc(a_addr + Cfg::A_BYTES, 8192, 1024, 2) : make_desc_sw128_kmajor(a_addr + Cfg::A_BYTES);
#pragma unroll
          for (int k = 0; k < BK / UMMA_K; ++k) {
            if (leader) umma_bf16(tmem_d, da + uint64_t(k * (A_MN ? 128 : 2)), db + uint64_t(k * (B_MN ? 128 : 2)), idesc, ((kb - kb0) | k) != 0 ? 1u : 0u);
          }
          if (leader) umma_commit(&empty_bar[s]);
        }
        if (leader) umma_commit(&acc_full[buf]);
        if (leader) gprof(4 + min(int(lt), 3));
      }
    }
  } else if (warp >= 4) {
    const int q = warp & 3;
    const int half = (warp - 4) >> 2;
    constexpr int HALF_COLS = BN / 2;
    drop = drop_resolve(drop);
    uint32_t lt = 0;
    for (int tile = blockIdx.x; tile < n_tiles; tile += gridDim.x, ++lt) {
      const int split = tile / mn_tiles, mn = tile - split * mn_tiles;
      const int m0 = (mn / n_blocks) * BM, n0 = (mn % n_blocks) * BN;
      OutT* Cs = C + size_t(split) * split_stride;
      const uint32_t buf = lt & 1, aph = (lt >> 1) & 1;
      const int row = m0 + q * 32 + lane;
      const uint32_t taddr = tmem_base + (uint32_t(q * 32) << 16) + buf * BN + half * HALF_COLS;
      const float* bias_t = bias;
      if (flags & AVF_EPI_BIAS) {
        float* bs = reinterpret_cast<float*>(smem + Cfg::BIAS_OFF) + buf * BN;
        for (int i = threadIdx.x - 128; i < BN; i += 256) bs[i] = __ldg(bias + n0 + i);
        asm volatile("bar.sync 1, 256;" ::: "memory");
        bias_t = bs - n0;
      }
      if constexpr (HALF_COLS <= 64) {
        float4 pre[HALF_COLS / 4];
        const bool want_res = (flags & AVF_EPI_RESIDUAL) != 0;
        if (want_res) {
#pragma unroll
          for (int j = 0; j < HALF_COLS / 16; ++j)
            quad_load16(res, ld_res, row, n0 + half * HALF_COLS + j * 16, M, lane, reinterpret_cast<float4(&)[4]>(pre[4 * j]));
        }
        mbar_wait(&acc_full[buf], aph);
        tc_fence_after();
        if (threadIdx.x == 128) gprof(8 + min(int(lt), 3));
#pragma unroll
        for (int c0 = 0; c0 < HALF_COLS; c0 += 32) {
          uint32_t v[32];
          tmem_ld32(taddr + uint32_t(c0), v);
          tmem_ld_wait();
          if (c0 + 32 >= HALF_COLS) {
            tc_fence_before();
            __syncwarp();
            if (lane == 0) mbar_arrive(&acc_empty[buf]);
          }
          epilogue_chunk<OutT>(v, row, n0 + half * HALF_COLS + c0, Cs, ldc, bias_t, res, ld_res, flags, aux, ld_aux, drop, N, M, want_res ? &pre[c0 / 4] : nullptr);
        }
      } else {
        mbar_wait(&acc_full[buf], aph);
        tc_fence_after();
        if (threadIdx.x == 128) gprof(8 + min(int(lt), 3));
#pragma unroll 1
        for (int c0 = 0; c0 < HALF_COLS; c0 += 32) {
          uint32_t v[32];
          tmem_ld32(taddr + uint32_t(c0), v);
          tmem_ld_wait();
          if (c0 + 32 >= HALF_COLS) {
            tc_fence_before();
            __syncwarp();
            if (lane == 0) mbar_arrive(&acc_empty[buf]);
          }
          epilogue_chunk<OutT>(v, row, n0 + half * HALF_COLS + c0, Cs, ldc, bias_t, res, ld_res, flags, aux, ld_aux, drop, N, M);
        }
      }
    }
  }

  if (threadIdx.x == 128) gprof(12);
  tc_fence_before();
  __syncthreads();
  if (warp == 2) tmem_dealloc(tmem_base, Cfg::TMEM_COLS);
  if (threadIdx.x == 0) gprof(13);
}

using EncodeTiledFn = CUresult (*)(CUtensorMap*, CUtensorMapDataType, cuuint32_t, void*, const cuuint64_t*,
                                   const cuuint64_t*, const cuuint32_t*, const cuuint32_t*, CUtensorMapInterleave,
                                   CUtensorMapSwizzle, CUtensorMapL2promotion, CUtensorMapFloatOOBfill);

EncodeTiledFn get_encode_fn() {
  static EncodeTiledFn fn = nullptr;
  static std::once_flag once;
  std::call_once(once, [] {
    void* p = nullptr;
    cudaDriverEntryPointQueryResult qres;
    if (cudaGetDriverEntryPoint("cuTensorMapEncodeTiled", &p, cudaEnableDefault, &qres) == cudaSuccess &&
        qres == cudaDriverEntryPointSuccess)
      fn = reinterpret_cast<EncodeTiledFn>(p);
  });
  return fn;
}

}

namespace {
struct TmapKey {
  const void* ptr;
  uint64_t rows, cols, ld;
  uint32_t box_rows, box_cols;
  bool operator==(const TmapKey& o) const {
    return ptr == o.ptr && rows == o.rows && cols == o.cols && ld == o.ld && box_rows == o.box_rows && box_cols == o.box_cols;
  }
};
struct TmapKeyHash {
  size_t operator()(const TmapKey& k) const {
    uint64_t h = reinterpret_cast<uintptr_t>(k.ptr) * 0x9E3779B97F4A7C15ull;
    h ^= (k.rows * 0xBF58476D1CE4E5B9ull) ^ (k.cols << 21) ^ (k.ld << 42) ^ (uint64_t(k.box_rows) << 7) ^ k.box_cols;
    return size_t(h ^ (h >> 29));
  }
};
constexpr size_t TMAP_CACHE_MAX = 4096;
std::atomic<uint64_t> g_tmap_hits{0}, g_tmap_misses{0};
}

void tmap_cache_stats(uint64_t* hits, uint64_t* misses) {
  *hits = g_tmap_hits.load();
  *misses = g_tmap_misses.load();
}

static int encode_tmap_bf16_2d(CUtensorMap* tm, const void* ptr, uint64_t rows, uint64_t cols, uint64_t ld, uint32_t box_rows, uint32_t box_cols);

int make_tmap_bf16_2d(CUtensorMap* tm, const void* ptr, uint64_t rows, uint64_t cols, uint64_t ld, uint32_t box_rows, uint32_t box_cols = 64) {
  static thread_local std::unordered_map<TmapKey, CUtensorMap, TmapKeyHash> cache;
  const TmapKey key{ptr, rows, cols, ld, box_rows, box_cols};
  auto it = cache.find(key);
  if (it != cache.end()) {
    *tm = it->second;
    g_tmap_hits.fetch_add(1, std::memory_order_relaxed);
    return 0;
  }
  const int e = encode_tmap_bf16_2d(tm, ptr, rows, cols, ld, box_rows, box_cols);
  if (e) return e;
  if (cache.size() >= TMAP_CACHE_MAX) cache.clear();
  cache.emplace(key, *tm);
  g_tmap_misses.fetch_add(1, std::memory_order_relaxed);
  return 0;
}

static int encode_tmap_bf16_2d(CUtensorMap* tm, const void* ptr, uint64_t rows, uint64_t cols, uint64_t ld, uint32_t box_rows, uint32_t box_cols) {
  EncodeTiledFn fn = get_encode_fn();
  AVF_REQUIRE(fn != nullptr, AVF_ENODEVICE, "cuTensorMapEncodeTiled is not available from the driver");
  AVF_REQUIRE((reinterpret_cast<uintptr_t>(ptr) & 15) == 0 && (ld * 2) % 16 == 0, AVF_EINVAL,
              "TMA operand must be 16-byte aligned with a 16-byte multiple row pitch (ptr=%p ld=%llu)", ptr,
              (unsigned long long)ld);
  cuuint64_t dims[2] = {cols, rows};
  cuuint64_t strides[1] = {ld * 2};
  AVF_REQUIRE(box_cols == 64 || box_cols == 32, AVF_EINVAL, "tensor map box must be 64 or 32 columns wide");
  cuuint32_t box[2] = {box_cols, box_rows};
  cuuint32_t estr[2] = {1, 1};
  CUresult r = fn(tm, CU_TENSOR_MAP_DATA_TYPE_BFLOAT16, 2, const_cast<void*>(ptr), dims, strides, box, estr,
                  CU_TENSOR_MAP_INTERLEAVE_NONE, box_cols == 64 ? CU_TENSOR_MAP_SWIZZLE_128B : CU_TENSOR_MAP_SWIZZLE_64B,
                  CU_TENSOR_MAP_L2_PROMOTION_L2_256B,
                  CU_TENSOR_MAP_FLOAT_OOB_FILL_NONE);
  AVF_REQUIRE(r == CUDA_SUCCESS, AVF_EINVAL, "cuTensorMapEncodeTiled failed with CUresult %d", int(r));
  return 0;
}

static int sm_count() { return sm_count_of_current_device(); }

template <int BN, int STAGES, typename OutT, bool A_MN, bool B_MN>
static int launch_gemm(const void* a, int lda, const void* w, int ldw, OutT* c, int ldc, const float* bias,
                       const float* res, int ld_res, int m, int n, int k, int flags, const void* aux, int ld_aux,
                       int splits, size_t split_stride, cudaStream_t stream, DropSpec drop = DropSpec{}) {
  using Cfg = GemmCfg<BN, STAGES>;
  CUtensorMap ta, tw;
  int e = A_MN ? make_tmap_bf16_2d(&ta, a, k, m, lda, 64) : make_tmap_bf16_2d(&ta, a, m, k, lda, BM);
  if (e) return e;
  e = B_MN ? make_tmap_bf16_2d(&tw, w, k, n, ldw, 64) : make_tmap_bf16_2d(&tw, w, n, k, ldw, BN);
  if (e) return e;
  auto kern = gemm_umma_kernel<BN, STAGES, OutT, A_MN, B_MN>;
  static PerDeviceOnce once;
  if (once.first()) AVF_CUDA(cudaFuncSetAttribute(kern, cudaFuncAttributeMaxDynamicSharedMemorySize, Cfg::SMEM_BYTES));
  const int n_tiles = (n / BN) * ceil_div(m, BM) * splits;
  const int cap = sm_cap();
  launch_pdl(kern, min(n_tiles, cap > 0 ? min(cap, sm_count()) : sm_count()), 384, Cfg::SMEM_BYTES, stream, ta, tw, c, ldc, bias, res, ld_res, m, n, k, flags,
                                                                   static_cast<__nv_bfloat16*>(const_cast<void*>(aux)), ld_aux, splits, split_stride, drop);
  AVF_LAUNCH_CHECK("gemm_umma_kernel");
  return 0;
}

namespace {
__global__ void __launch_bounds__(256) splitk_reduce_kernel(const float* __restrict__ part, int splits, size_t n, float* __restrict__ out,
                                                            int accumulate) {
  pdl_wait();
  pdl_trigger();
  const size_t i = (size_t(blockIdx.x) * blockDim.x + threadIdx.x) * 4;
  if (i >= n) return;
  float4 acc = *reinterpret_cast<const float4*>(part + i);
  if (accumulate) {
    const float4 v = *reinterpret_cast<const float4*>(out + i);
    acc.x += v.x; acc.y += v.y; acc.z += v.z; acc.w += v.w;
  }
  for (int s = 1; s < splits; ++s) {
    const float4 v = *reinterpret_cast<const float4*>(part + size_t(s) * n + i);
    acc.x += v.x; acc.y += v.y; acc.z += v.z; acc.w += v.w;
  }
  *reinterpret_cast<float4*>(out + i) = acc;
}
}

int gemm_umma(int trans_a, int trans_b, const void* a, int lda, const void* w, int ldw, const float* bias, const float* res,
              int ld_res, const void* aux, int ld_aux, void* c, int ldc, int c_mode, int m, int n, int k, int flags,
              void* ws, size_t ws_bytes, cudaStream_t stream, DropSpec drop) {
  AVF_REQUIRE(m > 0 && n > 0 && k > 0, AVF_EINVAL, "linear: empty problem m=%d n=%d k=%d", m, n, k);
  AVF_REQUIRE(n % 64 == 0, AVF_EUNSUPPORTED, "linear(bf16): N=%d must be a multiple of 64", n);
  AVF_REQUIRE(trans_a || trans_b || k % 8 == 0, AVF_EUNSUPPORTED, "linear(bf16): K=%d must be a multiple of 8", k);
  AVF_REQUIRE(!trans_a || m % 64 == 0, AVF_EUNSUPPORTED, "linear(bf16): M=%d of a transposed A must be a multiple of 64", m);
  AVF_REQUIRE(ldc % 8 == 0 && (!(flags & AVF_EPI_RESIDUAL) || ld_res % 4 == 0), AVF_EINVAL,
              "linear(bf16): ldc=%d / ld_res=%d break vector alignment", ldc, ld_res);
  AVF_REQUIRE(!(flags & (AVF_EPI_DGELU | AVF_EPI_SAVE_PRE)) || (aux != nullptr && ld_aux % 8 == 0), AVF_EINVAL,
              "linear(bf16): DGELU / SAVE_PRE epilogues need the pre-activation buffer");
  const int m_tiles = ceil_div(m, BM), sms = sm_count();
  if (trans_a && trans_b) {
    const bool accumulate = (flags & AVF_EPI_ACCUMULATE) != 0;
    AVF_REQUIRE(c_mode == AVF_FP32 && (flags & ~AVF_EPI_ACCUMULATE) == 0, AVF_EUNSUPPORTED, "linear(bf16): the TN form writes (or accumulates into) plain fp32");
    const int bn = n % 128 == 0 ? 128 : 64;
    const int mn_tiles = m_tiles * (n / bn), kblocks = ceil_div(k, BK);
    int splits = std::max(1, std::min(kblocks, sms / std::max(1, mn_tiles)));
    const int per = ceil_div(kblocks, splits);
    splits = ceil_div(kblocks, per);
    const size_t elems = size_t(m) * n;
    float* out = static_cast<float*>(c);
    float* part = out;
    size_t stride = 0;
    if (splits > 1 || accumulate) {
      AVF_REQUIRE(ldc == n, AVF_EINVAL, "linear(bf16): split-K output must be dense (ldc=%d n=%d)", ldc, n);
      AVF_REQUIRE(ws != nullptr && ws_bytes >= elems * splits * sizeof(float), AVF_EWORKSPACE,
                  "linear(bf16): split-K workspace too small: %zu < %zu bytes", ws_bytes, elems * splits * sizeof(float));
      part = static_cast<float*>(ws);
      stride = elems;
    }
    int e = bn == 128 ? launch_gemm<128, 6, float, true, true>(a, lda, w, ldw, part, ldc, nullptr, nullptr, 0, m, n, k, 0, nullptr, 0, splits, stride, stream)
                      : launch_gemm<64, 8, float, true, true>(a, lda, w, ldw, part, ldc, nullptr, nullptr, 0, m, n, k, 0, nullptr, 0, splits, stride, stream);
    if (e) return e;
    if (splits > 1 || accumulate) {
      launch_pdl(splitk_reduce_kernel, unsigned((elems / 4 + 255) / 256), 256, 0, stream, part, splits, elems, out, accumulate ? 1 : 0);
      AVF_LAUNCH_CHECK("splitk_reduce_kernel");
    }
    return 0;
  }
  AVF_REQUIRE(!trans_a, AVF_EUNSUPPORTED, "linear(bf16): transposed A is only implemented together with transposed B");
  int bn = 64;
  if (n % 256 == 0 && m_tiles * (n / 256) * 5 >= (c_mode == AVF_BF16 ? 4 : 10) * sms) bn = 256;
  else if (n % 128 == 0 && m_tiles * (n / 128) >= sms) bn = 128;
  else if (n % 128 == 0 && n / 128 * m_tiles >= sms / 2 && n >= 512) bn = 128;
#define AVF_GEMM(BN_, ST_, BMN_)                                                                                                   \
  if (bn == BN_ && bool(trans_b) == BMN_) {                                                                                        \
    if (c_mode == AVF_BF16)                                                                                                        \
      return launch_gemm<BN_, ST_, __nv_bfloat16, false, BMN_>(a, lda, w, ldw, static_cast<__nv_bfloat16*>(c), ldc, bias, res, ld_res, m, n, k, flags, aux, ld_aux, 1, 0, stream, drop); \
    return launch_gemm<BN_, ST_, float, false, BMN_>(a, lda, w, ldw, static_cast<float*>(c), ldc, bias, res, ld_res, m, n, k, flags, aux, ld_aux, 1, 0, stream, drop);          \
  }
  AVF_GEMM(256, 4, false)
  AVF_GEMM(128, 6, false)
  AVF_GEMM(64, 8, false)
  AVF_GEMM(256, 4, true)
  AVF_GEMM(128, 6, true)
  AVF_GEMM(64, 8, true)
#undef AVF_GEMM
  return AVF_EUNSUPPORTED;
}

int gemm_prof_read(unsigned long long* out16) {
#ifdef AVF_GEMM_PROF
  AVF_CUDA(cudaDeviceSynchronize());
  AVF_CUDA(cudaMemcpyFromSymbol(out16, g_gemm_prof, sizeof(unsigned long long) * 16));
  return 0;
#else
  (void)out16;
  return AVF_EUNSUPPORTED;
#endif
}

size_t gemm_umma_workspace_bytes(int m, int n, int k) {
  const int sms = sm_count(), bn = n % 128 == 0 ? 128 : 64;
  const int mn_tiles = ceil_div(m, BM) * (n / bn), kblocks = ceil_div(k, BK);
  const int splits = std::max(1, std::min(kblocks, sms / std::max(1, mn_tiles)));
  return size_t(m) * n * splits * sizeof(float);
}

int linear_umma(const void* a, int lda, const void* w, const float* bias, const float* res, int ld_res, void* c,
                int ldc, int c_mode, int m, int n, int k, int flags, cudaStream_t stream) {
  AVF_REQUIRE(k % BK == 0, AVF_EUNSUPPORTED, "linear(bf16): K=%d must be a multiple of %d", k, BK);
  return gemm_umma(0, 0, a, lda, w, k, bias, res, ld_res, nullptr, 0, c, ldc, c_mode, m, n, k, flags, nullptr, 0, stream, DropSpec{});
}

}
```

multi-modal-multi-label-facial-action-unit-detection-with-transformer_b200/csrc/avf_internal.h:

```cpp
#pragma once
#include <cuda_runtime.h>
#include <stddef.h>

#include "../../include/avformer_b200.h"
#include "avf_common.cuh"

namespace avf {

int layernorm(int out_mode, const float* x, int ld_x, const float* g, const float* b, void* y, int rows, int dim, cudaStream_t st);
int bn_rows(int out_mode, const float* x, int ld_x, const float* g, const float* b, const float* mean, const float* var, void* y,
            int rows, int dim, cudaStream_t st);
int sformer_pack(int io_mode, const void* fmap, const float* pos, float* x, int n_frames, int dim, int hw, cudaStream_t st);
int sformer_unpack(int io_mode, const float* x, void* fmap, int n_frames, int dim, int hw, cudaStream_t st);
int tformer_embed(int io_mode, const void* frames, const float* cls, const float* pos, float* x, int n_clips, int T, int dim, cudaStream_t st);
int tformer_embed_indexed(int io_mode, const void* bank, int n_bank, const int* index, const float* cls, const float* pos, float* x, uint8_t* keep,
                          int n_clips, int T, int dim, cudaStream_t st);
size_t tformer_embed_indexed_bwd_workspace_bytes(int n_clips, int T, int n_bank);
int tformer_embed_indexed_bwd(int out_mode, const float* dtok, const int* index, int n_clips, int T, int dim, int n_bank, void* dbank, void* ws,
                              size_t ws_bytes, cudaStream_t st);
int rows_gather(const float* x, size_t src_row_stride, float* y, int rows, int dim, cudaStream_t st);
int add_row_periodic(float* x, int ld_x, const float* pos, int rows, int dim, int period, cudaStream_t st);
int cast_f32_bf16(const float* s, void* d, size_t n, cudaStream_t st);
int cast_bf16_f32(const void* s, float* d, size_t n, cudaStream_t st);
int au_logits(const float* x, int ld_x, const float* w_last, float* out21, int* decisions, int n_clips, int dim, cudaStream_t st);
int au_bce(const float* logits, int ld, const float* labels, const float* pw, float* loss_out, float* dlogits, int n_clips, cudaStream_t st);
size_t peer_gather_bytes(int world, size_t n);
int logits_push(const float* logits, size_t n, const unsigned long long* peer_base, int world, int rank, const uint32_t* state, cudaStream_t st);
size_t peer_allreduce_bytes(int world, size_t n);
int grad_allreduce(const unsigned long long* peer_base, size_t n, int world, int rank, uint32_t* state, unsigned long long timeout_ns, cudaStream_t st);
int adam_allreduce_step(const unsigned long long* peer_base, size_t n, int world, int rank, uint32_t* state, unsigned long long timeout_ns, float* p, float* m,
                        float* v, void* shadow, float lr, float b1, float b2, float eps, float wd, int step, int decoupled, float grad_scale, cudaStream_t st);
int logits_wait(const void* my_base, size_t n, int world, uint32_t* state, unsigned long long timeout_ns, cudaStream_t st);
int au_confusion(const float* pred, int ld_pred, float thresh, const float* labels, int ld_lab, float ignore, unsigned long long* counts, int n_rows,
                 cudaStream_t st);

int linear_f32(const float* a, int lda, const float* w, const float* bias, const float* res, int ld_res, void* c, int ldc,
               int c_mode, int m, int n, int k, int flags, cudaStream_t st);
int attention_small(int io_mode, const void* qkv, void* out, int n_seq, int n_tok, int heads, int dim_head, cudaStream_t st,
                    const uint8_t* keep = nullptr);

int gemm_f32(int trans_a, int trans_b, const float* a, int lda, const float* w, int ldw, const float* bias, const float* res, int ld_res,
             float* aux, int ld_aux, void* c, int ldc, int c_mode, int m, int n, int k, int flags, cudaStream_t st, DropSpec drop = DropSpec{});

size_t colsum_workspace_bytes(int rows, int cols);
int colsum(int in_mode, const void* x, size_t ld, int rows, int cols, float* out, float beta, void* ws, size_t ws_bytes, cudaStream_t st);
size_t layernorm_bwd_workspace_bytes(int rows, int dim);
int layernorm_bwd(const float* x, int ld_x, const float* gamma, const float* dyn, float* dres, int ld_d, void* dxb, int dxb_mode, float* dgamma,
                  float* dbeta, float* dbias, float beta_acc, int rows, int dim, void* ws, size_t ws_bytes, cudaStream_t st,
                  DropSpec drop_in = DropSpec{}, DropSpec drop_out = DropSpec{});
int masked_copy(const float* x, void* y, int y_mode, int rows, int dim, DropSpec drop, cudaStream_t st);
int dropout_mask(float* out, int rows, int cols, DropSpec drop, cudaStream_t st);
int attention_bwd(int io_mode, const void* qkv, const void* dout, void* dqkv, int n_seq, int n_tok, int heads, int dim_head, cudaStream_t st,
                  const uint8_t* keep = nullptr);
int au_logits_bwd(const float* dl, int ld_dl, const float* x, int ld_x, const float* w_last, float* dx, int ld_dx, float* dw, int n_clips,
                  int dim, cudaStream_t st);
int bn_train_fwd(int out_mode, const float* x, int ld_x, const float* g, const float* b, float* run_mean, float* run_var, float momentum,
                 void* y, float* save_mean, float* save_rstd, int rows, int dim, cudaStream_t st);
int bn_bwd(const float* x, int ld_x, const float* dy, const float* g, const float* mean, const float* rstd_or_var, int batch_stats, float* dx,
           int ld_dx, float* dgamma, float* dbeta, int rows, int dim, cudaStream_t st);
int adam_step(float* p, const float* g, float* m, float* v, void* shadow, size_t n, float lr, float b1, float b2, float eps, float wd, int step,
              int decoupled, float grad_scale, cudaStream_t st);

int attention_mma_bf16(const void* qkv, void* out, int n_seq, int n_tok, int heads, int dim_head, cudaStream_t st, int q_rows = 0,
                       const uint8_t* keep = nullptr);
int attention_bwd_mma_bf16(const void* qkv, const void* dout, void* dqkv, int n_seq, int n_tok, int heads, int dim_head, cudaStream_t st,
                           const uint8_t* keep = nullptr);

bool encoder_fused_supported(const avf_stack_shape* s);
int fused_prof_read(unsigned long long* out64, int reset);
int fused_set_trap_buffer(void* host_mapped_words);
size_t encoder_fused_scratch_bytes();
int encoder_fused(int io_kind, const avf_stack_shape* s, const avf_layer_weights* L, const void* in, int ld_in, void* out, int ld_out,
                  const float* pos, void* scratch, const float* w_last, float* out21, int* decisions, cudaStream_t st);

int gemm_umma(int trans_a, int trans_b, const void* a, int lda, const void* w, int ldw, const float* bias, const float* res, int ld_res,
              const void* aux, int ld_aux, void* c, int ldc, int c_mode, int m, int n, int k, int flags, void* ws, size_t ws_bytes,
              cudaStream_t stream, DropSpec drop = DropSpec{});
size_t gemm_umma_workspace_bytes(int m, int n, int k);
void tmap_cache_stats(uint64_t* hits, uint64_t* misses);
int gemm_prof_read(unsigned long long* out16);
int linear_umma(const void* a, int lda, const void* w, const float* bias, const float* res, int ld_res, void* c, int ldc,
                int c_mode, int m, int n, int k, int flags, cudaStream_t st);

}
```

Before: 486,400.

## Fuse QKV projection GEMM with attention in tcgen05 GEMM epilogue

Adds a variant of the UMMA GEMM kernel whose epilogue warps run small-sequence attention directly on the QKV tile. Per-head Q/K/V columns are loaded together and staged in shared memory, so the QKV intermediate never goes through global memory and one launch per layer is removed. The last layer's residual gather is also folded into the out-projection by reading the residual with a strided ld. The cost is a more complex kernel with extra shared memory and attention work serialized inside the GEMM epilogue.

```diff
diff --git a/multi-modal-multi-label-facial-action-unit-detection-with-transformer_b200/csrc/avf_api.cu b/multi-modal-multi-label-facial-action-unit-detection-with-transformer_b200/csrc/avf_api.cu
--- a/multi-modal-multi-label-facial-action-unit-detection-with-transformer_b200/csrc/avf_api.cu
+++ b/multi-modal-multi-label-facial-action-unit-detection-with-transformer_b200/csrc/avf_api.cu
@@ -112,6 +112,10 @@
          ld_x % 4 == 0 && (out == nullptr || ld_out % 4 == 0);
 }
 
+static bool fused_qkv_attention(int mode, const avf_stack_shape* s) {
+  return mode == AVF_BF16 && g_fused.load() && tcgen05_ok() && qkv_attention_supported(s->n_tok, s->dim_head, s->dim);
+}
+
 static int encoder_stack(int mode, const avf_stack_shape* s, const avf_layer_weights* L, float* x, int ld_x, float* out, int ld_out,
                          void* ws, size_t ws_bytes, cudaStream_t st, const uint8_t* keep = nullptr) {
   int e = check_shape(s);
@@ -123,11 +127,16 @@
   const EncoderWs w = carve_encoder_ws(s, mode, ws);
   AVF_REQUIRE(ws_bytes >= w.total, AVF_EWORKSPACE, "workspace too small: %zu < %zu bytes", ws_bytes, w.total);
   const int R = s->n_seq * s->n_tok, D = s->dim, I = s->heads * s->dim_head, M = s->mlp_dim;
+  const bool qkv_att = fused_qkv_attention(mode, s);
   for (int l = 0; l < s->depth; ++l) {
     const avf_layer_weights& W = L[l];
     if ((e = layernorm(mode, x, ld_x, W.ln1_gamma, W.ln1_beta, w.ln, R, D, st))) return e;
-    if ((e = linear(mode, w.ln, D, W.w_qkv, nullptr, nullptr, 0, w.qkv, 3 * I, mode, R, 3 * I, D, 0, st))) return e;
-    if ((e = attention_small(mode, w.qkv, w.attn, s->n_seq, s->n_tok, s->heads, s->dim_head, st, keep))) return e;
+    if (qkv_att) {
+      if ((e = qkv_attention(w.ln, W.w_qkv, w.attn, s->n_seq, s->n_tok, s->heads, D, 0, keep, st))) return e;
+    } else {
+      if ((e = linear(mode, w.ln, D, W.w_qkv, nullptr, nullptr, 0, w.qkv, 3 * I, mode, R, 3 * I, D, 0, st))) return e;
+      if ((e = attention_small(mode, w.qkv, w.attn, s->n_seq, s->n_tok, s->heads, s->dim_head, st, keep))) return e;
+    }
     if ((e = linear(mode, w.attn, I, W.w_out, W.b_out, x, ld_x, x, ld_x, AVF_FP32, R, D, I, AVF_EPI_BIAS | AVF_EPI_RESIDUAL, st))) return e;
     if ((e = layernorm(mode, x, ld_x, W.ln2_gamma, W.ln2_beta, w.ln, R, D, st))) return e;
     if ((e = linear(mode, w.ln, D, W.w_ff1, W.b_ff1, nullptr, 0, w.hid, M, mode, R, M, D, AVF_EPI_BIAS | AVF_EPI_GELU, st))) return e;
@@ -169,15 +178,17 @@
   }
   const avf_layer_weights& W = layers[s->depth - 1];
   if ((e = layernorm(mode, x, D, W.ln1_gamma, W.ln1_beta, w.ln, R, D, st))) return e;
-  if ((e = linear(mode, w.ln, D, W.w_qkv, nullptr, nullptr, 0, w.qkv, 3 * I, mode, R, 3 * I, D, 0, st))) return e;
-  if (mode == AVF_BF16) {
+  if (fused_qkv_attention(mode, s)) {
+    if ((e = qkv_attention(w.ln, W.w_qkv, oc, B, N, s->heads, D, 1, keep, st))) return e;
+  } else if (mode == AVF_BF16) {
+    if ((e = linear(mode, w.ln, D, W.w_qkv, nullptr, nullptr, 0, w.qkv, 3 * I, mode, R, 3 * I, D, 0, st))) return e;
     if ((e = attention_mma_bf16(w.qkv, oc, B, N, s->heads, s->dim_head, st, 1, keep))) return e;
   } else {
+    if ((e = linear(mode, w.ln, D, W.w_qkv, nullptr, nullptr, 0, w.qkv, 3 * I, mode, R, 3 * I, D, 0, st))) return e;
     if ((e = attention_small(mode, w.qkv, w.attn, B, N, s->heads, s->dim_head, st, keep))) return e;
     AVF_CUDA(cudaMemcpy2DAsync(oc, size_t(I) * 4, w.attn, size_t(N) * I * 4, size_t(I) * 4, B, cudaMemcpyDeviceToDevice, st));
   }
-  if ((e = rows_gather(x, size_t(N) * D, xc, B, D, st))) return e;
-  if ((e = linear(mode, oc, I, W.w_out, W.b_out, xc, D, xc, D, AVF_FP32, B, D, I, AVF_EPI_BIAS | AVF_EPI_RESIDUAL, st))) return e;
+  if ((e = linear(mode, oc, I, W.w_out, W.b_out, x, N * D, xc, D, AVF_FP32, B, D, I, AVF_EPI_BIAS | AVF_EPI_RESIDUAL, st))) return e;
   if ((e = layernorm(mode, xc, D, W.ln2_gamma, W.ln2_beta, lnc, B, D, st))) return e;
   if ((e = linear(mode, lnc, D, W.w_ff1, W.b_ff1, nullptr, 0, hc, M, mode, B, M, D, AVF_EPI_BIAS | AVF_EPI_GELU, st))) return e;
   return linear(mode, hc, M, W.w_ff2, W.b_ff2, xc, D, cls_out, D, AVF_FP32, B, D, M, AVF_EPI_BIAS | AVF_EPI_RESIDUAL, st);
diff --git a/multi-modal-multi-label-facial-action-unit-detection-with-transformer_b200/csrc/avf_attention_core.cuh b/multi-modal-multi-label-facial-action-unit-detection-with-transformer_b200/csrc/avf_attention_core.cuh
--- /dev/null
+++ b/multi-modal-multi-label-facial-action-unit-detection-with-transformer_b200/csrc/avf_attention_core.cuh
@@ -0,0 +1,129 @@
+#pragma once
+#include "avf_common.cuh"
+
+namespace avf {
+
+__device__ __forceinline__ void mma_bf16_16816(float (&d)[4], const uint32_t (&a)[4], uint32_t b0, uint32_t b1) {
+  asm volatile(
+      "mma.sync.aligned.m16n8k16.row.col.f32.bf16.bf16.f32 {%0,%1,%2,%3}, {%4,%5,%6,%7}, {%8,%9}, {%0,%1,%2,%3};"
+      : "+f"(d[0]), "+f"(d[1]), "+f"(d[2]), "+f"(d[3])
+      : "r"(a[0]), "r"(a[1]), "r"(a[2]), "r"(a[3]), "r"(b0), "r"(b1));
+}
+
+__device__ __forceinline__ void ldmatrix_x2_trans(uint32_t& r0, uint32_t& r1, const void* smem_row_ptr) {
+  asm volatile("ldmatrix.sync.aligned.m8n8.x2.trans.shared.b16 {%0,%1}, [%2];" : "=r"(r0), "=r"(r1) : "r"(smem_u32(smem_row_ptr)));
+}
+
+__device__ __forceinline__ void quad_transpose32(uint32_t (&p)[4], int lane) {
+  const bool b0 = lane & 1, b1 = lane & 2;
+  uint32_t r;
+  r = __shfl_xor_sync(0xffffffffu, b0 ? p[0] : p[1], 1); if (b0) p[0] = r; else p[1] = r;
+  r = __shfl_xor_sync(0xffffffffu, b0 ? p[2] : p[3], 1); if (b0) p[2] = r; else p[3] = r;
+  r = __shfl_xor_sync(0xffffffffu, b1 ? p[0] : p[2], 2); if (b1) p[0] = r; else p[2] = r;
+  r = __shfl_xor_sync(0xffffffffu, b1 ? p[1] : p[3], 2); if (b1) p[1] = r; else p[3] = r;
+}
+
+__device__ __forceinline__ uint64_t keep_bits(const uint8_t* __restrict__ row, int n_tok, int lane) {
+  const uint32_t lo = __ballot_sync(0xffffffffu, lane < n_tok && row[lane] != 0);
+  const uint32_t hi = __ballot_sync(0xffffffffu, lane + 32 < n_tok && row[lane + 32] != 0);
+  return (uint64_t(hi) << 32) | lo;
+}
+
+__device__ __forceinline__ float mask_score(float s, bool row_kept, uint64_t km, int c, int n_tok) {
+  if (c >= n_tok) return -INFINITY;
+  if (!row_kept) return 0.f;
+  return ((km >> c) & 1) ? s : -INFINITY;
+}
+
+template <int DH, int NP, bool MASKED, int PITCH, typename KV, typename LoadQ>
+__device__ __forceinline__ void attention_warp(LoadQ&& load_q, KV (*Ks)[PITCH], KV (*Vs)[PITCH], uint64_t km, int n_tok, int q_rows,
+                                               float scale_log2e, __nv_bfloat16* __restrict__ out, int seq, int head, int inner, int lane) {
+  const int g = lane >> 2, t = lane & 3;
+#pragma unroll 1
+  for (int mt = 0; mt < NP / 16; ++mt) {
+    if (mt * 16 >= q_rows) break;
+    const int r_lo = mt * 16 + g, r_hi = r_lo + 8;
+    uint32_t qf[DH / 16][4];
+    load_q(qf, r_lo, r_hi);
+    float s[NP / 8][4];
+#pragma unroll
+    for (int nt = 0; nt < NP / 8; ++nt) {
+      s[nt][0] = s[nt][1] = s[nt][2] = s[nt][3] = 0.f;
+#pragma unroll
+      for (int ks = 0; ks < DH / 16; ++ks) {
+        const uint32_t b0 = *reinterpret_cast<const uint32_t*>(&Ks[nt * 8 + g][ks * 16 + 2 * t]);
+        const uint32_t b1 = *reinterpret_cast<const uint32_t*>(&Ks[nt * 8 + g][ks * 16 + 8 + 2 * t]);
+        mma_bf16_16816(s[nt], qf[ks], b0, b1);
+      }
+    }
+    float m_lo = -INFINITY, m_hi = -INFINITY;
+    const bool k_lo = (km >> r_lo) & 1, k_hi = (km >> r_hi) & 1;
+#pragma unroll
+    for (int nt = 0; nt < NP / 8; ++nt) {
+      const int c = nt * 8 + 2 * t;
+      if constexpr (MASKED) {
+        s[nt][0] = mask_score(s[nt][0], k_lo, km, c, n_tok); s[nt][1] = mask_score(s[nt][1], k_lo, km, c + 1, n_tok);
+        s[nt][2] = mask_score(s[nt][2], k_hi, km, c, n_tok); s[nt][3] = mask_score(s[nt][3], k_hi, km, c + 1, n_tok);
+      } else {
+        if (c >= n_tok) { s[nt][0] = -INFINITY; s[nt][2] = -INFINITY; }
+        if (c + 1 >= n_tok) { s[nt][1] = -INFINITY; s[nt][3] = -INFINITY; }
+      }
+      m_lo = fmaxf(m_lo, fmaxf(s[nt][0], s[nt][1]));
+      m_hi = fmaxf(m_hi, fmaxf(s[nt][2], s[nt][3]));
+    }
+    m_lo = fmaxf(m_lo, __shfl_xor_sync(0xffffffffu, m_lo, 1));
+    m_lo = fmaxf(m_lo, __shfl_xor_sync(0xffffffffu, m_lo, 2));
+    m_hi = fmaxf(m_hi, __shfl_xor_sync(0xffffffffu, m_hi, 1));
+    m_hi = fmaxf(m_hi, __shfl_xor_sync(0xffffffffu, m_hi, 2));
+    const float o_lo = m_lo * scale_log2e, o_hi = m_hi * scale_log2e;
+    float l_lo = 0.f, l_hi = 0.f;
+#pragma unroll
+    for (int nt = 0; nt < NP / 8; ++nt) {
+      s[nt][0] = exp2f(fmaf(s[nt][0], scale_log2e, -o_lo));
+      s[nt][1] = exp2f(fmaf(s[nt][1], scale_log2e, -o_lo));
+      s[nt][2] = exp2f(fmaf(s[nt][2], scale_log2e, -o_hi));
+      s[nt][3] = exp2f(fmaf(s[nt][3], scale_log2e, -o_hi));
+      l_lo += s[nt][0] + s[nt][1];
+      l_hi += s[nt][2] + s[nt][3];
+    }
+    l_lo += __shfl_xor_sync(0xffffffffu, l_lo, 1);
+    l_lo += __shfl_xor_sync(0xffffffffu, l_lo, 2);
+    l_hi += __shfl_xor_sync(0xffffffffu, l_hi, 1);
+    l_hi += __shfl_xor_sync(0xffffffffu, l_hi, 2);
+    float o[DH / 8][4];
+#pragma unroll
+    for (int nt = 0; nt < DH / 8; ++nt) o[nt][0] = o[nt][1] = o[nt][2] = o[nt][3] = 0.f;
+#pragma unroll
+    for (int kt = 0; kt < NP / 16; ++kt) {
+      uint32_t pa[4];
+      pa[0] = pack_bf16x2(s[2 * kt][0], s[2 * kt][1]);
+      pa[1] = pack_bf16x2(s[2 * kt][2], s[2 * kt][3]);
+      pa[2] = pack_bf16x2(s[2 * kt + 1][0], s[2 * kt + 1][1]);
+      pa[3] = pack_bf16x2(s[2 * kt + 1][2], s[2 * kt + 1][3]);
+#pragma unroll
+      for (int nt = 0; nt < DH / 8; ++nt) {
+        uint32_t b0, b1;
+        ldmatrix_x2_trans(b0, b1, &Vs[kt * 16 + (lane & 15)][nt * 8]);
+        mma_bf16_16816(o[nt], pa, b0, b1);
+      }
+    }
+    const float i_lo = 1.f / l_lo, i_hi = 1.f / l_hi;
+    __nv_bfloat16* olo = out + (size_t(seq) * q_rows + r_lo) * inner + head * DH;
+    __nv_bfloat16* ohi = out + (size_t(seq) * q_rows + r_hi) * inner + head * DH;
+#pragma unroll
+    for (int grp = 0; grp < DH / 32; ++grp) {
+      uint32_t lo[4], hi[4];
+#pragma unroll
+      for (int j = 0; j < 4; ++j) {
+        lo[j] = pack_bf16x2(o[grp * 4 + j][0] * i_lo, o[grp * 4 + j][1] * i_lo);
+        hi[j] = pack_bf16x2(o[grp * 4 + j][2] * i_hi, o[grp * 4 + j][3] * i_hi);
+      }
+      quad_transpose32(lo, lane);
+      quad_transpose32(hi, lane);
+      if (r_lo < q_rows) *reinterpret_cast<uint4*>(olo + (grp * 4 + t) * 8) = make_uint4(lo[0], lo[1], lo[2], lo[3]);
+      if (r_hi < q_rows) *reinterpret_cast<uint4*>(ohi + (grp * 4 + t) * 8) = make_uint4(hi[0], hi[1], hi[2], hi[3]);
+    }
+  }
+}
+
+}
diff --git a/multi-modal-multi-label-facial-action-unit-detection-with-transformer_b200/csrc/avf_attention_mma.cu b/multi-modal-multi-label-facial-action-unit-detection-with-transformer_b200/csrc/avf_attention_mma.cu
--- a/multi-modal-multi-label-facial-action-unit-detection-with-transformer_b200/csrc/avf_attention_mma.cu
+++ b/multi-modal-multi-label-facial-action-unit-detection-with-transformer_b200/csrc/avf_attention_mma.cu
@@ -1,41 +1,10 @@
+#include "avf_attention_core.cuh"
 #include "avf_common.cuh"
 #include "avf_internal.h"
 
 namespace avf {
 
 namespace {
-
-__device__ __forceinline__ void mma_bf16_16816(float (&d)[4], const uint32_t (&a)[4], uint32_t b0, uint32_t b1) {
-  asm volatile(
-      "mma.sync.aligned.m16n8k16.row.col.f32.bf16.bf16.f32 {%0,%1,%2,%3}, {%4,%5,%6,%7}, {%8,%9}, {%0,%1,%2,%3};"
-      : "+f"(d[0]), "+f"(d[1]), "+f"(d[2]), "+f"(d[3])
-      : "r"(a[0]), "r"(a[1]), "r"(a[2]), "r"(a[3]), "r"(b0), "r"(b1));
-}
-
-__device__ __forceinline__ void ldmatrix_x2_trans(uint32_t& r0, uint32_t& r1, const void* smem_row_ptr) {
-  asm volatile("ldmatrix.sync.aligned.m8n8.x2.trans.shared.b16 {%0,%1}, [%2];" : "=r"(r0), "=r"(r1) : "r"(smem_u32(smem_row_ptr)));
-}
-
-__device__ __forceinline__ void quad_transpose32(uint32_t (&p)[4], int lane) {
-  const bool b0 = lane & 1, b1 = lane & 2;
-  uint32_t r;
-  r = __shfl_xor_sync(0xffffffffu, b0 ? p[0] : p[1], 1); if (b0) p[0] = r; else p[1] = r;
-  r = __shfl_xor_sync(0xffffffffu, b0 ? p[2] : p[3], 1); if (b0) p[2] = r; else p[3] = r;
-  r = __shfl_xor_sync(0xffffffffu, b1 ? p[0] : p[2], 2); if (b1) p[0] = r; else p[2] = r;
-  r = __shfl_xor_sync(0xffffffffu, b1 ? p[1] : p[3], 2); if (b1) p[1] = r; else p[3] = r;
-}
-
-__device__ __forceinline__ uint64_t keep_bits(const uint8_t* __restrict__ row, int n_tok, int lane) {
-  const uint32_t lo = __ballot_sync(0xffffffffu, lane < n_tok && row[lane] != 0);
-  const uint32_t hi = __ballot_sync(0xffffffffu, lane + 32 < n_tok && row[lane + 32] != 0);
-  return (uint64_t(hi) << 32) | lo;
-}
-
-__device__ __forceinline__ float mask_score(float s, bool row_kept, uint64_t km, int c, int n_tok) {
-  if (c >= n_tok) return -INFINITY;
-  if (!row_kept) return 0.f;
-  return ((km >> c) & 1) ? s : -INFINITY;
-}
 
 template <int DH, int NP, bool MASKED>
 __global__ void __launch_bounds__(DH == 32 ? 128 : 64) attention_mma_kernel(const __nv_bfloat16* __restrict__ qkv, __nv_bfloat16* __restrict__ out,
@@ -81,12 +50,8 @@
   }
   __syncwarp();
 
-  const int g = lane >> 2, t = lane & 3;
-#pragma unroll 1
-  for (int mt = 0; mt < NP / 16; ++mt) {
-    if (mt * 16 >= q_rows) break;
-    const int r_lo = mt * 16 + g, r_hi = r_lo + 8;
-    uint32_t qf[DH / 16][4];
+  const int t = lane & 3;
+  auto load_q = [&](uint32_t (&qf)[DH / 16][4], int r_lo, int r_hi) {
 #pragma unroll
     for (int grp = 0; grp < DH / 32; ++grp) {
       uint32_t lo[4] = {0u, 0u, 0u, 0u}, hi[4] = {0u, 0u, 0u, 0u};
@@ -107,85 +72,8 @@
         qf[ks][half * 2 + 1] = hi[j];
       }
     }
-    float s[NP / 8][4];
-#pragma unroll
-    for (int nt = 0; nt < NP / 8; ++nt) {
-      s[nt][0] = s[nt][1] = s[nt][2] = s[nt][3] = 0.f;
-#pragma unroll
-      for (int ks = 0; ks < DH / 16; ++ks) {
-        const uint32_t b0 = *reinterpret_cast<const uint32_t*>(&Ks[nt * 8 + g][ks * 16 + 2 * t]);
-        const uint32_t b1 = *reinterpret_cast<const uint32_t*>(&Ks[nt * 8 + g][ks * 16 + 8 + 2 * t]);
-        mma_bf16_16816(s[nt], qf[ks], b0, b1);
-      }
-    }
-    float m_lo = -INFINITY, m_hi = -INFINITY;
-    const bool k_lo = (km >> r_lo) & 1, k_hi = (km >> r_hi) & 1;
-#pragma unroll
-    for (int nt = 0; nt < NP / 8; ++nt) {
-      const int c = nt * 8 + 2 * t;
-      if constexpr (MASKED) {
-        s[nt][0] = mask_score(s[nt][0], k_lo, km, c, n_tok); s[nt][1] = mask_score(s[nt][1], k_lo, km, c + 1, n_tok);
-        s[nt][2] = mask_score(s[nt][2], k_hi, km, c, n_tok); s[nt][3] = mask_score(s[nt][3], k_hi, km, c + 1, n_tok);
-      } else {
-        if (c >= n_tok) { s[nt][0] = -INFINITY; s[nt][2] = -INFINITY; }
-        if (c + 1 >= n_tok) { s[nt][1] = -INFINITY; s[nt][3] = -INFINITY; }
-      }
-      m_lo = fmaxf(m_lo, fmaxf(s[nt][0], s[nt][1]));
-      m_hi = fmaxf(m_hi, fmaxf(s[nt][2], s[nt][3]));
-    }
-    m_lo = fmaxf(m_lo, __shfl_xor_sync(0xffffffffu, m_lo, 1));
-    m_lo = fmaxf(m_lo, __shfl_xor_sync(0xffffffffu, m_lo, 2));
-    m_hi = fmaxf(m_hi, __shfl_xor_sync(0xffffffffu, m_hi, 1));
-    m_hi = fmaxf(m_hi, __shfl_xor_sync(0xffffffffu, m_hi, 2));
-    const float o_lo = m_lo * scale_log2e, o_hi = m_hi * scale_log2e;
-    float l_lo = 0.f, l_hi = 0.f;
-#pragma unroll
-    for (int nt = 0; nt < NP / 8; ++nt) {
-      s[nt][0] = exp2f(fmaf(s[nt][0], scale_log2e, -o_lo));
-      s[nt][1] = exp2f(fmaf(s[nt][1], scale_log2e, -o_lo));
-      s[nt][2] = exp2f(fmaf(s[nt][2], scale_log2e, -o_hi));
-      s[nt][3] = exp2f(fmaf(s[nt][3], scale_log2e, -o_hi));
-      l_lo += s[nt][0] + s[nt][1];
-      l_hi += s[nt][2] + s[nt][3];
-    }
-    l_lo += __shfl_xor_sync(0xffffffffu, l_lo, 1);
-    l_lo += __shfl_xor_sync(0xffffffffu, l_lo, 2);
-    l_hi += __shfl_xor_sync(0xffffffffu, l_hi, 1);
-    l_hi += __shfl_xor_sync(0xffffffffu, l_hi, 2);
-    float o[DH / 8][4];
-#pragma unroll
-    for (int nt = 0; nt < DH / 8; ++nt) o[nt][0] = o[nt][1] = o[nt][2] = o[nt][3] = 0.f;
-#pragma unroll
-    for (int kt = 0; kt < NP / 16; ++kt) {
-      uint32_t pa[4];
-      pa[0] = pack_bf16x2(s[2 * kt][0], s[2 * kt][1]);
-      pa[1] = pack_bf16x2(s[2 * kt][2], s[2 * kt][3]);
-      pa[2] = pack_bf16x2(s[2 * kt + 1][0], s[2 * kt + 1][1]);
-      pa[3] = pack_bf16x2(s[2 * kt + 1][2], s[2 * kt + 1][3]);
-#pragma unroll
-      for (int nt = 0; nt < DH / 8; ++nt) {
-        uint32_t b0, b1;
-        ldmatrix_x2_trans(b0, b1, &Vs[kt * 16 + (lane & 15)][nt * 8]);
-        mma_bf16_16816(o[nt], pa, b0, b1);
-      }
-    }
-    const float i_lo = 1.f / l_lo, i_hi = 1.f / l_hi;
-    __nv_bfloat16* olo = out + (size_t(seq) * q_rows + r_lo) * inner + head * DH;
-    __nv_bfloat16* ohi = out + (size_t(seq) * q_rows + r_hi) * inner + head * DH;
-#pragma unroll
-    for (int grp = 0; grp < DH / 32; ++grp) {
-      uint32_t lo[4], hi[4];
-#pragma unroll
-      for (int j = 0; j < 4; ++j) {
-        lo[j] = pack_bf16x2(o[grp * 4 + j][0] * i_lo, o[grp * 4 + j][1] * i_lo);
-        hi[j] = pack_bf16x2(o[grp * 4 + j][2] * i_hi, o[grp * 4 + j][3] * i_hi);
-      }
-      quad_transpose32(lo, lane);
-      quad_transpose32(hi, lane);
-      if (r_lo < q_rows) *reinterpret_cast<uint4*>(olo + (grp * 4 + t) * 8) = make_uint4(lo[0], lo[1], lo[2], lo[3]);
-      if (r_hi < q_rows) *reinterpret_cast<uint4*>(ohi + (grp * 4 + t) * 8) = make_uint4(hi[0], hi[1], hi[2], hi[3]);
-    }
-  }
+  };
+  attention_warp<DH, NP, MASKED, PITCH>(load_q, Ks, Vs, km, n_tok, q_rows, scale_log2e, out, seq, head, inner, lane);
 }
 
 template <int DH, int NP, bool MASKED>
diff --git a/multi-modal-multi-label-facial-action-unit-detection-with-transformer_b200/csrc/avf_gemm_umma.cu b/multi-modal-multi-label-facial-action-unit-detection-with-transformer_b200/csrc/avf_gemm_umma.cu
--- a/multi-modal-multi-label-facial-action-unit-detection-with-transformer_b200/csrc/avf_gemm_umma.cu
+++ b/multi-modal-multi-label-facial-action-unit-detection-with-transformer_b200/csrc/avf_gemm_umma.cu
@@ -6,6 +6,7 @@
 #include <algorithm>
 #include <mutex>
 
+#include "avf_attention_core.cuh"
 #include "avf_common.cuh"
 
 namespace avf {
@@ -24,8 +25,21 @@
   static constexpr int BAR_OFF = STAGES * STAGE_BYTES;
   static constexpr int BIAS_OFF = BAR_OFF + 256;
   static constexpr int SMEM_BYTES = BIAS_OFF + 2 * BN * 4 + 1024;
-  static constexpr int TMEM_COLS = 2 * BN;
+  static constexpr int TMEM_COLS = 2 * BN > 256 ? 512 : 2 * BN;
 };
+
+struct AttEpi {
+  __nv_bfloat16* out = nullptr;
+  const uint8_t* keep = nullptr;
+  int n_seq = 0, n_tok = 0, spb = 0, q_rows = 0;
+  float scale_log2e = 0.f;
+};
+constexpr int ATT_BN = 192, ATT_STAGES = 4;
+constexpr int ATT_PITCH = ATT_BN + 8;
+constexpr int ATT_ROWS = 144;
+constexpr int ATT_STAGE_OFF = GemmCfg<ATT_BN, ATT_STAGES>::BIAS_OFF + 2 * ATT_BN * 4;
+constexpr int ATT_SMEM_BYTES = ATT_STAGE_OFF + ATT_ROWS * ATT_PITCH * 2 + 1024;
+static_assert(ATT_SMEM_BYTES <= 227 * 1024, "operand ring + staged tile exceed the shared memory of a block");
 
 __device__ __forceinline__ void quad_transpose(uint4 (&p)[4], int lane) {
   auto xchg = [&](uint4& keep_lo, uint4& keep_hi, bool upper, int mask) {
@@ -160,12 +174,69 @@
 __device__ __forceinline__ void gprof(int) {}
 #endif
 
-template <int BN, int STAGES, typename OutT, bool A_MN, bool B_MN>
+template <int NP>
+__device__ __forceinline__ void attention_epilogue(uint8_t* smem, uint64_t* acc_full, uint64_t* acc_empty, uint32_t tmem_base, const AttEpi& att,
+                                                   int n_tiles, int n_blocks, int N, int warp, int lane) {
+  constexpr int BN = ATT_BN;
+  using StageRow = __nv_bfloat16[ATT_PITCH];
+  StageRow* stg = reinterpret_cast<StageRow*>(smem + ATT_STAGE_OFF);
+  for (int i = threadIdx.x - 128; i < (ATT_ROWS - BM) * ATT_PITCH / 8; i += 256)
+    reinterpret_cast<uint4*>(stg[BM])[i] = make_uint4(0u, 0u, 0u, 0u);
+  const int q = warp & 3, half = (warp - 4) >> 2, ew = warp - 4;
+  const int n_tok = att.n_tok, inner = N / 3, t = lane & 3;
+  uint32_t lt = 0;
+  for (int tile = blockIdx.x; tile < n_tiles; tile += gridDim.x, ++lt) {
+    const int seq0 = (tile / n_blocks) * att.spb, head = tile % n_blocks;
+    const uint32_t buf = lt & 1, aph = (lt >> 1) & 1;
+    const uint32_t taddr = tmem_base + (uint32_t(q * 32) << 16) + buf * BN + half * (BN / 2);
+    mbar_wait(&acc_full[buf], aph);
+    tc_fence_after();
+#pragma unroll
+    for (int c0 = 0; c0 < BN / 2; c0 += 32) {
+      uint32_t v[32];
+      tmem_ld32(taddr + uint32_t(c0), v);
+      tmem_ld_wait();
+      if (c0 + 32 >= BN / 2) {
+        tc_fence_before();
+        __syncwarp();
+        if (lane == 0) mbar_arrive(&acc_empty[buf]);
+      }
+      uint4* dst = reinterpret_cast<uint4*>(&stg[q * 32 + lane][half * (BN / 2) + c0]);
+#pragma unroll
+      for (int j = 0; j < 4; ++j)
+        dst[j] = make_uint4(pack_bf16x2(__uint_as_float(v[8 * j]), __uint_as_float(v[8 * j + 1])),
+                            pack_bf16x2(__uint_as_float(v[8 * j + 2]), __uint_as_float(v[8 * j + 3])),
+                            pack_bf16x2(__uint_as_float(v[8 * j + 4]), __uint_as_float(v[8 * j + 5])),
+                            pack_bf16x2(__uint_as_float(v[8 * j + 6]), __uint_as_float(v[8 * j + 7])));
+    }
+    asm volatile("bar.sync 1, 256;" ::: "memory");
+    const int n_here = min(att.spb, att.n_seq - seq0);
+    for (int p = ew; p < n_here; p += 8) {
+      StageRow* Qs = stg + p * n_tok;
+      const uint64_t km = att.keep != nullptr ? keep_bits(att.keep + size_t(seq0 + p) * n_tok, n_tok, lane)
+                                              : (n_tok == 64 ? ~0ull : (1ull << n_tok) - 1);
+      auto load_q = [&](uint32_t (&qf)[4][4], int r_lo, int r_hi) {
+#pragma unroll
+        for (int ks = 0; ks < 4; ++ks) {
+          qf[ks][0] = *reinterpret_cast<const uint32_t*>(&Qs[r_lo][ks * 16 + 2 * t]);
+          qf[ks][1] = *reinterpret_cast<const uint32_t*>(&Qs[r_hi][ks * 16 + 2 * t]);
+          qf[ks][2] = *reinterpret_cast<const uint32_t*>(&Qs[r_lo][ks * 16 + 8 + 2 * t]);
+          qf[ks][3] = *reinterpret_cast<const uint32_t*>(&Qs[r_hi][ks * 16 + 8 + 2 * t]);
+        }
+      };
+      attention_warp<64, NP, true, ATT_PITCH>(load_q, reinterpret_cast<StageRow*>(&Qs[0][64]), reinterpret_cast<StageRow*>(&Qs[0][128]), km,
+                                                  n_tok, att.q_rows, att.scale_log2e, att.out, seq0 + p, head, inner, lane);
+    }
+    asm volatile("bar.sync 1, 256;" ::: "memory");
+  }
+}
+
+template <int BN, int STAGES, typename OutT, bool A_MN, bool B_MN, int ATT_NP = 0>
 __global__ void __launch_bounds__(384, 1)
 gemm_umma_kernel(const __grid_constant__ CUtensorMap tm_a, const __grid_constant__ CUtensorMap tm_w,
                  OutT* C, int ldc, const float* __restrict__ bias,
                  const float* res, int ld_res, int M, int N, int K, int flags,
-                 __nv_bfloat16* aux, int ld_aux, int splits, size_t split_stride, DropSpec drop) {
+                 __nv_bfloat16* aux, int ld_aux, int splits, size_t split_stride, DropSpec drop, AttEpi att) {
   using Cfg = GemmCfg<BN, STAGES>;
   extern __shared__ uint8_t smem_raw[];
   uint8_t* smem = reinterpret_cast<uint8_t*>((reinterpret_cast<uintptr_t>(smem_raw) + 1023) & ~uintptr_t(1023));
@@ -180,7 +251,8 @@
   const int kblocks_total = (K + BK - 1) / BK;
   const int kb_per_split = (kblocks_total + splits - 1) / splits;
   const int n_blocks = N / BN;
-  const int mn_tiles = n_blocks * ((M + BM - 1) / BM);
+  const int m_step = ATT_NP > 0 ? att.spb * att.n_tok : BM;
+  const int mn_tiles = n_blocks * (ATT_NP > 0 ? (att.n_seq + att.spb - 1) / att.spb : (M + BM - 1) / BM);
   const int n_tiles = mn_tiles * splits;
 
   if (warp == 0 && lane == 0) {
@@ -215,7 +287,7 @@
       uint32_t it = 0;
       for (int tile = blockIdx.x; tile < n_tiles; tile += gridDim.x) {
         const int split = tile / mn_tiles, mn = tile - split * mn_tiles;
-        const int m0 = (mn / n_blocks) * BM, n0 = (mn % n_blocks) * BN;
+        const int m0 = (mn / n_blocks) * m_step, n0 = (mn % n_blocks) * BN;
         const int kb0 = split * kb_per_split, kb1 = min(kblocks_total, kb0 + kb_per_split);
         for (int kb = kb0; kb < kb1; ++kb, ++it) {
           const int s = it % STAGES;
@@ -230,7 +302,10 @@
             } else {
               tma_load_2d(st, &tm_a, &full_bar[s], kb * BK, m0);
             }
-            if constexpr (B_MN) {
+            if constexpr (ATT_NP > 0) {
+#pragma unroll
+              for (int p = 0; p < 3; ++p) tma_load_2d(st + Cfg::A_BYTES + p * 8192, &tm_w, &full_bar[s], kb * BK, p * (N / 3) + (mn % n_blocks) * 64);
+            } else if constexpr (B_MN) {
 #pragma unroll
               for (int p = 0; p < BN / 64; ++p) tma_load_2d(st + Cfg::A_BYTES + p * 8192, &tm_w, &full_bar[s], n0 + p * 64, kb * BK);
             } else {
@@ -272,6 +347,8 @@
         if (leader) gprof(4 + min(int(lt), 3));
       }
     }
+  } else if (ATT_NP > 0 && warp >= 4) {
+    if constexpr (ATT_NP > 0) attention_epilogue<ATT_NP>(smem, acc_full, acc_empty, tmem_base, att, n_tiles, n_blocks, N, warp, lane);
   } else if (warp >= 4) {
     const int q = warp & 3;
     const int half = (warp - 4) >> 2;
@@ -442,7 +519,7 @@
   const int n_tiles = (n / BN) * ceil_div(m, BM) * splits;
   const int cap = sm_cap();
   launch_pdl(kern, min(n_tiles, cap > 0 ? min(cap, sm_count()) : sm_count()), 384, Cfg::SMEM_BYTES, stream, ta, tw, c, ldc, bias, res, ld_res, m, n, k, flags,
-                                                                   static_cast<__nv_bfloat16*>(const_cast<void*>(aux)), ld_aux, splits, split_stride, drop);
+                                                                   static_cast<__nv_bfloat16*>(const_cast<void*>(aux)), ld_aux, splits, split_stride, drop, AttEpi{});
   AVF_LAUNCH_CHECK("gemm_umma_kernel");
   return 0;
 }
@@ -546,6 +623,47 @@
   return size_t(m) * n * splits * sizeof(float);
 }
 
+template <int NP>
+static int launch_qkv_attention(const CUtensorMap& ta, const CUtensorMap& tw, int m, int n, int k, const AttEpi& att, int n_tiles, cudaStream_t st) {
+  auto kern = gemm_umma_kernel<ATT_BN, ATT_STAGES, __nv_bfloat16, false, false, NP>;
+  static PerDeviceOnce once;
+  if (once.first()) AVF_CUDA(cudaFuncSetAttribute(kern, cudaFuncAttributeMaxDynamicSharedMemorySize, ATT_SMEM_BYTES));
+  const int cap = sm_cap();
+  launch_pdl(kern, min(n_tiles, cap > 0 ? min(cap, sm_count()) : sm_count()), 384, ATT_SMEM_BYTES, st, ta, tw, static_cast<__nv_bfloat16*>(nullptr), 0,
+             static_cast<const float*>(nullptr), static_cast<const float*>(nullptr), 0, m, n, k, 0, static_cast<__nv_bfloat16*>(nullptr), 0, 1, size_t(0),
+             DropSpec{}, att);
+  AVF_LAUNCH_CHECK("gemm_umma_kernel (attention epilogue)");
+  return 0;
+}
+
+bool qkv_attention_supported(int n_tok, int dim_head, int dim) { return n_tok >= 1 && n_tok <= 64 && dim_head == 64 && dim % BK == 0; }
+
+int qkv_attention(const void* a, const void* w_qkv, void* out, int n_seq, int n_tok, int heads, int dim, int q_rows, const uint8_t* keep,
+                  cudaStream_t st) {
+  AVF_REQUIRE(n_seq > 0 && heads > 0 && qkv_attention_supported(n_tok, 64, dim), AVF_EUNSUPPORTED,
+              "qkv_attention: n_seq=%d n_tok=%d heads=%d dim=%d (1..64 tokens, 64-wide heads, dim a multiple of %d)", n_seq, n_tok, heads, dim, BK);
+  const int inner = heads * 64, m = n_seq * n_tok;
+  CUtensorMap ta, tw;
+  int e = make_tmap_bf16_2d(&ta, a, m, dim, dim, BM);
+  if (e) return e;
+  if ((e = make_tmap_bf16_2d(&tw, w_qkv, 3 * inner, dim, dim, 64))) return e;
+  AttEpi att;
+  att.out = static_cast<__nv_bfloat16*>(out);
+  att.keep = keep;
+  att.n_seq = n_seq;
+  att.n_tok = n_tok;
+  att.spb = BM / n_tok;
+  att.q_rows = (q_rows <= 0 || q_rows > n_tok) ? n_tok : q_rows;
+  att.scale_log2e = 1.4426950408889634f / sqrtf(64.f);
+  const int n_tiles = ceil_div(n_seq, att.spb) * heads;
+  switch ((n_tok + 15) / 16) {
+    case 1: return launch_qkv_attention<16>(ta, tw, m, 3 * inner, dim, att, n_tiles, st);
+    case 2: return launch_qkv_attention<32>(ta, tw, m, 3 * inner, dim, att, n_tiles, st);
+    case 3: return launch_qkv_attention<48>(ta, tw, m, 3 * inner, dim, att, n_tiles, st);
+    default: return launch_qkv_attention<64>(ta, tw, m, 3 * inner, dim, att, n_tiles, st);
+  }
+}
+
 int linear_umma(const void* a, int lda, const void* w, const float* bias, const float* res, int ld_res, void* c,
                 int ldc, int c_mode, int m, int n, int k, int flags, cudaStream_t stream) {
   AVF_REQUIRE(k % BK == 0, AVF_EUNSUPPORTED, "linear(bf16): K=%d must be a multiple of %d", k, BK);
diff --git a/multi-modal-multi-label-facial-action-unit-detection-with-transformer_b200/csrc/avf_internal.h b/multi-modal-multi-label-facial-action-unit-detection-with-transformer_b200/csrc/avf_internal.h
--- a/multi-modal-multi-label-facial-action-unit-detection-with-transformer_b200/csrc/avf_internal.h
+++ b/multi-modal-multi-label-facial-action-unit-detection-with-transformer_b200/csrc/avf_internal.h
@@ -81,5 +81,8 @@
 int gemm_prof_read(unsigned long long* out16);
 int linear_umma(const void* a, int lda, const void* w, const float* bias, const float* res, int ld_res, void* c, int ldc,
                 int c_mode, int m, int n, int k, int flags, cudaStream_t st);
+bool qkv_attention_supported(int n_tok, int dim_head, int dim);
+int qkv_attention(const void* a, const void* w_qkv, void* out, int n_seq, int n_tok, int heads, int dim, int q_rows, const uint8_t* keep,
+                  cudaStream_t st);
 
 }
```

Measured after the change: 492,600, median of 6. +1.3%, better.
